# mlelarge/graph_neural_net

Measured on AMD Instinct MI355X. Metric: graph-pairs/sec FGNN fwd+bwd, N=50 regular pairs, higher is better.
Workload: dtype f32

## Files before the change

### graph_neural_net_amd/_lib.py

```python
import ctypes as C
import os

import torch

_HERE = os.path.dirname(os.path.abspath(__file__))
LIB_PATH = os.environ.get('FGNN_LIB') or os.path.join(_HERE, 'libfgnn_hip.so')

FGNN_H = 32
FGNN_TILE = 32
FGNN_MAX_DEPTH = 3
FGNN_RANGE_WG = 256
FGNN_LSAP_MAX_N = 2048
FGNN_QAP_MAX_N = 256
FGNN_SPECTRAL_MAX_N = 256
FGNN_SPECTRAL_MAX_POWERS = 8
FGNN_SCORE_SPLIT = 4

c_float_p = C.c_void_p


class Slab(C.Structure):
    _fields_ = [('ptr', C.c_void_p), ('gstride', C.c_longlong), ('ldp', C.c_longlong), ('C', C.c_int),
                ('nrm', C.c_void_p), ('beta', C.c_void_p)]


class MlpFwdArgs(C.Structure):
    _fields_ = [('G', C.c_int), ('N', C.c_int), ('depth', C.c_int), ('nmlp', C.c_int),
                ('nvalid', C.c_void_p),
                ('a', Slab), ('b', Slab),
                ('W', (C.c_void_p * FGNN_MAX_DEPTH) * 2),
                ('bias', (C.c_void_p * FGNN_MAX_DEPTH) * 2),
                ('z', C.c_void_p * 2),
                ('ldz', C.c_longlong),
                ('part', C.c_void_p * 2),
                ('cnt', C.c_void_p), ('packed', C.c_void_p), ('xbits', C.c_void_p), ('xdeg', C.c_void_p),
                ('ranges', C.c_void_p), ('cu_share', C.c_int)]


class DwJob(C.Structure):
    _fields_ = [('dy', C.c_void_p), ('d_gstride', C.c_longlong), ('d_ld', C.c_longlong), ('relu_mask', C.c_void_p),
                ('x', C.c_void_p), ('x_gstride', C.c_longlong), ('x_ld', C.c_longlong), ('M', C.c_int), ('K', C.c_int)]


class ChainLayer(C.Structure):
    _fields_ = [('W', C.c_void_p), ('w_ostride', C.c_longlong), ('w_kstride', C.c_longlong), ('bias', C.c_void_p),
                ('M', C.c_int), ('K', C.c_int), ('relu', C.c_int), ('mask', C.c_void_p), ('out', C.c_void_p),
                ('o_gstride', C.c_longlong)]


class ChainArgs(C.Structure):
    _fields_ = [('x', C.c_void_p), ('x_gstride', C.c_longlong), ('x_ld', C.c_longlong), ('depth', C.c_int),
                ('layer', ChainLayer * 3), ('o_ld', C.c_longlong), ('nvalid', C.c_void_p), ('G', C.c_int), ('N', C.c_int)]


class Mlp64Args(C.Structure):
    _fields_ = [('x', C.c_void_p), ('x_gstride', C.c_longlong), ('x_ld', C.c_longlong), ('cin', C.c_int),
                ('xb', C.c_void_p), ('xb_gstride', C.c_longlong), ('xb_ld', C.c_longlong), ('cb', C.c_int),
                ('packed', C.c_void_p), ('nvalid', C.c_void_p), ('G', C.c_int), ('N', C.c_int),
                ('out', C.c_void_p), ('o_gstride', C.c_longlong), ('o_ld', C.c_longlong),
                ('dz', C.c_void_p), ('dz_gstride', C.c_longlong), ('dz_ld', C.c_longlong),
                ('dx', C.c_void_p), ('dx_gstride', C.c_longlong), ('dx_ld', C.c_longlong),
                ('dxb', C.c_void_p), ('dxb_gstride', C.c_longlong), ('dxb_ld', C.c_longlong),
                ('accumulate_dx', C.c_int), ('accumulate_dxb', C.c_int),
                ('wpart', C.c_void_p)]


class Mlp64PackJob(C.Structure):
    _fields_ = [('W', C.c_void_p * 3), ('bias', C.c_void_p * 3), ('cin', C.c_int), ('packed', C.c_void_p)]


class MlpBwdArgs(C.Structure):
    _fields_ = [('G', C.c_int), ('N', C.c_int), ('depth', C.c_int),
                ('nvalid', C.c_void_p),
                ('a', Slab), ('b', Slab),
                ('W', C.c_void_p * FGNN_MAX_DEPTH),
                ('bias', C.c_void_p * FGNN_MAX_DEPTH),
                ('dy', C.c_void_p), ('dgstride', C.c_longlong), ('ldd', C.c_longlong),
                ('z', C.c_void_p), ('zgstride', C.c_longlong), ('ldz', C.c_longlong),
                ('coef', C.c_void_p), ('s12', C.c_void_p), ('znrm', C.c_void_p),
                ('dxa', C.c_void_p), ('dxa_gstride', C.c_longlong), ('dxa_ld', C.c_longlong),
                ('dxb', C.c_void_p), ('dxb_gstride', C.c_longlong), ('dxb_ld', C.c_longlong),
                ('accumulate_a', C.c_int), ('accumulate_b', C.c_int),
                ('wpart', C.c_void_p), ('s12part', C.c_void_p), ('packed', C.c_void_p),
                ('s12tiles', C.c_void_p), ('s12_out', C.c_void_p), ('xbits', C.c_void_p), ('xdeg', C.c_void_p),
                ('ranges', C.c_void_p), ('cu_share', C.c_int)]


class Slab16(C.Structure):
    _fields_ = [('ptr', C.c_void_p), ('gstride', C.c_longlong), ('ldp', C.c_longlong), ('C', C.c_int),
                ('nrm', C.c_void_p), ('beta', C.c_void_p)]


class MlpFwd16Args(C.Structure):
    _fields_ = [('G', C.c_int), ('N', C.c_int), ('ldr', C.c_int), ('depth', C.c_int), ('nmlp', C.c_int),
                ('nvalid', C.c_void_p),
                ('a', Slab16), ('b', Slab16),
                ('z', C.c_void_p * 2), ('ldz', C.c_longlong),
                ('part', C.c_void_p * 2), ('cnt', C.c_void_p), ('packed', C.c_void_p), ('ranges', C.c_void_p)]


class MlpBwd16Args(C.Structure):
    _fields_ = [('G', C.c_int), ('N', C.c_int), ('ldr', C.c_int), ('depth', C.c_int),
                ('nvalid', C.c_void_p),
                ('a', Slab16), ('b', Slab16),
                ('dy', C.c_void_p), ('dgstride', C.c_longlong), ('ldd', C.c_longlong),
                ('z', C.c_void_p), ('zgstride', C.c_longlong), ('ldz', C.c_longlong),
                ('coef', C.c_void_p),
                ('dxa', C.c_void_p), ('dxa_gstride', C.c_longlong), ('dxa_ld', C.c_longlong),
                ('dxb', C.c_void_p), ('dxb_gstride', C.c_longlong), ('dxb_ld', C.c_longlong),
                ('accumulate_a', C.c_int), ('accumulate_b', C.c_int),
                ('wpart', C.c_void_p), ('s12part', C.c_void_p), ('packed', C.c_void_p), ('ranges', C.c_void_p)]


class GradJob(C.Structure):
    _fields_ = [('wpart', C.c_void_p), ('count', C.c_int), ('out', C.c_void_p), ('s12', C.c_void_p),
                ('nrm', C.c_void_p), ('dgn_w', C.c_void_p), ('dgn_b', C.c_void_p), ('rows', C.c_int), ('scale', C.c_float), ('scale_dev', C.c_void_p)]


class PackJob(C.Structure):
    _fields_ = [('kind', C.c_int), ('ca', C.c_int), ('cb', C.c_int), ('depth', C.c_int), ('nmlp', C.c_int),
                ('W', (C.c_void_p * FGNN_MAX_DEPTH) * 2), ('bias', (C.c_void_p * FGNN_MAX_DEPTH) * 2),
                ('out', C.c_void_p)]


class PairgenArgs(C.Structure):
    _fields_ = [('seed', C.c_ulonglong), ('first', C.c_longlong), ('B', C.c_int), ('N', C.c_int),
                ('family', C.c_int), ('noise_model', C.c_int), ('edge_density', C.c_double),
                ('thr_edge', C.c_ulonglong), ('thr_noise1', C.c_ulonglong), ('thr_noise2', C.c_ulonglong),
                ('thr_vertex', C.c_ulonglong), ('swaps_per_edge', C.c_int),
                ('bits1', C.c_void_p), ('bits2', C.c_void_p), ('nvalid', C.c_void_p)]


MAX_GRAD_JOBS = 16
MAX_PACK_JOBS = 24
_VP, _LL, _I, _F = C.c_void_p, C.c_longlong, C.c_int, C.c_float

_SIGNATURES = {
    'fgnn_last_error': [],
    'fgnn_version': [],
    'fgnn_tiles_per_graph': [_I],
    'fgnn_mlp_bwd_num_workgroups': [],
    'fgnn_pack_floats': [_I, _I, _I, _I, _I],
    'fgnn_pack_operands': [_VP, _I, _VP],
    'fgnn_mlp_fwd': [C.POINTER(MlpFwdArgs), _VP],
    'fgnn_pack_x3_floats': [_I, _I, _I, _I, _I],
    'fgnn_pack_x3_operands': [_VP, _I, _VP],
    'fgnn_mlp_fwd_x3': [C.POINTER(MlpFwdArgs), _VP],
    'fgnn_debug_mlp_fwd_masks': [C.POINTER(MlpFwdArgs), _VP, _VP, _VP],
    'fgnn_debug_mlp_fwd_x3_masks': [C.POINTER(MlpFwdArgs), _VP, _VP, _VP],
    'fgnn_debug_matmul_variant': [_I],
    'fgnn_gn_finalize': [_VP, _VP, _VP, _VP, _I, _I, _I, _F, _VP, _VP],
    'fgnn_gn_finalize2': [_VP, _VP, _VP, _VP, _VP, _VP, _I, _I, _I, _F, _VP, _VP, _VP],
    'fgnn_gn_plane_supported': [_I],
    'fgnn_gn_plane_fwd': [_VP, _LL, _LL, _VP, _VP, _VP, _I, _I, _I, _F, _VP, _LL, _LL, _VP, _VP],
    'fgnn_gn_plane_bwd': [_VP, _LL, _LL, _VP, _LL, _LL, _VP, _VP, _I, _I, _I, _VP, _LL, _LL, _VP, _VP, _VP, _VP],
    'fgnn_gn_stats': [_VP, _LL, _LL, _VP, _VP, _I, _I, _I, _F, _VP, _VP],
    'fgnn_gn_apply': [_VP, _LL, _LL, _VP, _VP, _VP, _I, _I, _I, _VP, _LL, _LL, _VP],
    'fgnn_ragged_tile_ranges': [_VP, _I, _I, _VP, _VP],
    'fgnn_ragged_tile_ranges_order': [_VP, _I, _I, _VP, _VP, _VP],
    'fgnn_ragged_tile_ranges16': [_VP, _I, _I, _I, _VP, _VP],
    'fgnn_conv1x1_dw_multi': [C.POINTER(DwJob), _I, _VP, _I, _I, _VP, _VP],
    'fgnn_conv_chain_supported': [_I, _I, C.POINTER(C.c_int)],
    'fgnn_conv_chain': [C.POINTER(ChainArgs), _VP],
    'fgnn_mlp64_supported': [_I, _I, _I],
    'fgnn_mlp64_num_workgroups': [],
    'fgnn_mlp64_param_count': [_I],
    'fgnn_mlp64_packed_floats': [_I],
    'fgnn_mlp64_pack': [_VP, _VP, _VP, _VP, _VP, _VP, _I, _VP, _VP],
    'fgnn_mlp64_pack_multi': [C.POINTER(Mlp64PackJob), _I, _VP],
    'fgnn_mlp64_fwd': [C.POINTER(Mlp64Args), _VP],
    'fgnn_mlp64_bwd': [C.POINTER(Mlp64Args), _VP],
    'fgnn_conv1x1': [_VP, _LL, _LL, _VP, _VP, _LL, _LL, _VP, _I, _VP, _I, _I, _I, _I, _VP, _LL, _LL, _VP],
    'fgnn_conv1x1_dw_chunks': [_I, _I],
    'fgnn_conv1x1_dw': [_VP, _LL, _LL, _VP, _VP, _LL, _LL, _VP, _I, _I, _I, _I, _VP, _VP],
    'fgnn_chan_matmul_fwd': [C.POINTER(Slab), C.POINTER(Slab), _VP, _I, _I, _VP, _LL, _LL, _VP],
    'fgnn_chan_matmul_fwd_ord': [C.POINTER(Slab), C.POINTER(Slab), _VP, _I, _I, _VP, _LL, _LL, _VP, _I, _VP],
    'fgnn_chan_matmul_fwd_fin_supported': [_I],
    'fgnn_chan_matmul_fwd_fin': [C.POINTER(Slab), C.POINTER(Slab), _VP, _VP, _VP, _VP, _VP, _F, _VP, _I, _I, _VP, _LL, _LL, _VP],
    'fgnn_chan_matmul_fwd_fin_ord': [C.POINTER(Slab), C.POINTER(Slab), _VP, _VP, _VP, _VP, _VP, _F, _VP, _I, _I, _VP, _LL, _LL, _VP, _I, _VP],
    'fgnn_colmax_fwd': [C.POINTER(Slab), _VP, _I, _I, _VP, _VP, _VP],
    'fgnn_colmax_fwd_fin_supported': [_I],
    'fgnn_colmax_fwd_fin': [C.POINTER(Slab), _VP, _VP, _VP, _F, _VP, _I, _I, _VP, _VP, _VP],
    'fgnn_score_ce_fwd': [_VP, _VP, _VP, _I, _I, _I, _VP, _VP, _VP, _VP],
    'fgnn_score_row_blocks': [_I, _I],
    'fgnn_score_ce_fwd_blocks': [_VP, _VP, _VP, _I, _I, _I, _I, _VP, _VP, _VP, _VP],
    'fgnn_score_ce_bwd': [_VP, _VP, _VP, _VP, _VP, _VP, _I, _I, _I, _VP, _VP, _VP],
    'fgnn_inv_node_count': [_VP, _I, _VP, _VP],
    'fgnn_score_bwd': [_VP, _VP, _VP, _VP, _I, _I, _I, _VP, _VP, _VP],
    'fgnn_ce_fwd': [_VP, _VP, _I, _I, _VP, _VP, _VP],
    'fgnn_ce_bwd': [_VP, _VP, _VP, _VP, _I, _I, _VP, _VP],
    'fgnn_colmax_bwd': [_VP, _VP, _VP, _I, _I, _I, _VP, _LL, _LL, C.POINTER(Slab), _VP, _VP],
    'fgnn_gn_bwd_stats': [_VP, _LL, _LL, _VP, _LL, _LL, _VP, _VP, _I, _I, _I, _VP, _VP],
    'fgnn_gn_bwd_coef': [_VP, _VP, _VP, _I, _I, _I, _VP, _VP, _VP, _VP],
    'fgnn_gn_bwd_coef_tiles': [_VP, _VP, _VP, _I, _I, _I, _VP, _VP, _VP],
    'fgnn_grad_finalize': [_VP, _I, _I, _I, _I, _VP],
    'fgnn_gn_bwd_apply': [_VP, _LL, _LL, _VP, _LL, _LL, _VP, _VP, _I, _I, _I, _VP, _LL, _LL, _VP],
    'fgnn_mlp_bwd': [C.POINTER(MlpBwdArgs), _VP],
    'fgnn_mlp_bwd_x3': [C.POINTER(MlpBwdArgs), _VP],
    'fgnn_mlp_bwd_pair': [C.POINTER(MlpBwdArgs), C.POINTER(MlpBwdArgs), _VP],
    'fgnn_mlp_bwd_t16': [C.POINTER(MlpBwdArgs), _VP],
    'fgnn_mlp_bwd_t16_supported': [C.POINTER(MlpBwdArgs)],
    'fgnn_mlp_bwd_pair_t16': [C.POINTER(MlpBwdArgs), C.POINTER(MlpBwdArgs), _VP],
    'fgnn_mlp_bwd_pair_x3': [C.POINTER(MlpBwdArgs), C.POINTER(MlpBwdArgs), _VP],
    'fgnn_block1_struct_supported': [_I, _I, _I],
    'fgnn_block1_struct_table_floats': [_I],
    'fgnn_block1_struct_ws_floats': [_I, _I],
    'fgnn_block1_struct_rows': [_I, _I],
    'fgnn_block1_struct_fwd': [_VP, _VP, _I, _I, _VP, _VP, _VP, _VP, _VP, C.c_float, _VP, _VP, _VP, _LL, _LL, _VP, _VP, _VP, _VP, _VP, _VP, _VP],
    'fgnn_block1_struct_bwd': [_VP, _VP, _I, _I, _VP, _VP, _VP, _VP, _VP, _VP, _VP, _VP, _LL, _LL, _VP, _VP, _VP, _VP, _VP, _VP],
    'fgnn_block1_struct_fwd_pack': [_VP, _VP, _I, _I, _VP, _VP, _VP, _VP, _VP, C.c_float, _VP, _VP, _VP, _LL, _LL, _VP, _VP, _VP, _VP, _VP, _VP, _VP, _I, _VP],
    'fgnn_block1_struct_fwd16_pack': [_VP, _VP, _I, _I, _I, _VP, _VP, _VP, _VP, _VP, C.c_float, _VP, _VP, _VP, _LL, _LL, _VP, _VP, _VP, _VP, _VP, _VP, _VP, _I, _VP],
    'fgnn_block1_struct_fwd16': [_VP, _VP, _I, _I, _I, _VP, _VP, _VP, _VP, _VP, C.c_float, _VP, _VP, _VP, _LL, _LL, _VP, _VP, _VP, _VP, _VP, _VP, _VP],
    'fgnn_block1_struct_bwd16': [_VP, _VP, _I, _I, _I, _VP, _VP, _VP, _VP, _VP, _VP, _VP, _VP, _LL, _LL, _VP, _VP, _VP, _VP, _VP, _VP],
    'fgnn_mlp_bwd_coef_tiles_supported': [_I, _I],
    'fgnn_mlp_param_count': [_I, _I],
    'fgnn_reduce_partials': [_VP, _I, _I, _VP, _VP],
    'fgnn_chan_matmul_bwd': [C.POINTER(Slab), C.POINTER(Slab), _VP, _LL, _LL, _VP, _I, _I, _VP, _VP, _LL, _LL, _VP, _VP, _VP],
    'fgnn_chan_matmul_bwd_ord': [C.POINTER(Slab), C.POINTER(Slab), _VP, _LL, _LL, _VP, _I, _I, _VP, _VP, _LL, _LL, _VP, _VP, _VP, _I, _VP],
    'fgnn_sum_scale': [_VP, _I, _I, _F, _VP, _VP],
    'fgnn_adam_step': [_VP, _VP, _VP, _VP, _I, C.c_double, C.c_double, C.c_double, C.c_double, _I, C.c_double, _VP],
    'fgnn_adam_step_dev': [_VP, _VP, _VP, _VP, _I, _VP, _VP, _VP],
    'fgnn_expand_adjacency': [_VP, _VP, _I, _I, _VP, _VP],
    'fgnn_pack_adjacency': [_VP, _VP, _I, _I, _VP, _VP, _VP],
    'fgnn_pack_adjacency_ld': [_VP, _VP, _I, _I, _I, _VP, _VP, _VP],
    'fgnn_pack_adjacency_pair': [_VP, _VP, _VP, _VP, _I, _I, _I, _VP, _VP, _VP, _VP, _VP],
    'fgnn_adjacency_degree': [_VP, _VP, _I, _I, _VP, _VP],
    'fgnn_accuracy_max': [_VP, _VP, _I, _I, _VP, _VP],
    'fgnn_lsap_accuracy': [_VP, _LL, _I, _VP, _I, _I, _VP, _VP, _VP],
    'fgnn_pairgen_supported': [_I, _I, _I],
    'fgnn_pairgen': [C.POINTER(PairgenArgs), _VP],
    'fgnn_qap_objective': [_VP, _VP, _VP, _VP, _I, _I, _VP, _VP, _VP, _VP, _VP],
    'fgnn_qap_improve_cost': [_VP, _VP, _VP, _VP, _I, _I, _VP, _LL, _I, _VP],
    'fgnn_greedy_qap_ws_bytes': [_I, _I],
    'fgnn_greedy_qap': [_VP, _VP, _VP, _VP, _I, _I, _I, _VP, _LL, _VP, _VP, _VP, _VP, _VP],
    'fgnn_spectral_features': [_VP, _VP, _I, _I, _I, _VP, _I, _VP],
    'fgnn_tiles_per_graph16': [_I, _I],
    'fgnn_to_bf16': [_VP, _VP, _I, _I, _I, _I, _VP, _LL, _LL, _VP],
    'fgnn_from_bf16': [_VP, _LL, _LL, _I, _I, _I, _I, _VP, _VP],
    'fgnn_pack16_floats': [_I, _I, _I, _I, _I],
    'fgnn_pack16_operands': [_VP, _I, _VP],
    'fgnn_mlp_fwd16': [C.POINTER(MlpFwd16Args), _VP],
    'fgnn_debug_mlp_fwd16_masks': [C.POINTER(MlpFwd16Args), _VP, _VP, _VP],
    'fgnn_gn_finalize_tpg': [_VP, _VP, _VP, _VP, _I, _I, _I, _I, _F, _VP, _VP],
    'fgnn_gn_finalize2_tpg': [_VP, _VP, _VP, _VP, _VP, _VP, _I, _I, _I, _I, _F, _VP, _VP, _VP],
    'fgnn_gn_bwd_coef_tiles_tpg': [_VP, _VP, _VP, _I, _I, _I, _I, _VP, _VP, _VP],
    'fgnn_chan_matmul_fwd16': [C.POINTER(Slab16), C.POINTER(Slab16), _VP, _I, _I, _I, _VP, _LL, _LL, _VP],
    'fgnn_chan_matmul_fwd16_fin': [C.POINTER(Slab16), C.POINTER(Slab16), _VP, _VP, _VP, _VP, _VP, _F, _I, _VP, _I, _I, _I, _VP, _LL,
                                   _LL, _VP],
    'fgnn_chan_matmul_bwd16': [C.POINTER(Slab16), C.POINTER(Slab16), _VP, _LL, _LL, _VP, _I, _I, _I, _VP, _VP, _LL, _LL, _VP, _VP, _VP],
    'fgnn_chan_matmul_bwd16_t': [C.POINTER(Slab16), C.POINTER(Slab16), _VP, _LL, _LL, _VP, _I, _VP, _I, _I, _I, _VP, _VP, _LL, _LL,
                                 _VP, _VP, _VP],
    'fgnn_chan_matmul_bwd16_tc': [C.POINTER(Slab16), C.POINTER(Slab16), _VP, _LL, _LL, _VP, _I, _VP, _I, _I, _I, _VP, _VP, _LL, _LL,
                                  _VP, _VP, _VP, _VP, _VP],
    'fgnn_colmax_bwd16_coef': [_VP, _VP, _VP, _I, _I, _I, _I, _VP, _LL, _LL, C.POINTER(Slab16), _VP, _VP, _VP],
    'fgnn_colmax_fwd16': [C.POINTER(Slab16), _VP, _I, _I, _I, _VP, _VP, _VP],
    'fgnn_colmax_bwd16': [_VP, _VP, _VP, _I, _I, _I, _I, _VP, _LL, _LL, C.POINTER(Slab16), _VP, _VP],
    'fgnn_mlp_bwd16': [C.POINTER(MlpBwd16Args), _VP],
    'fgnn_mlp_bwd16_pair': [C.POINTER(MlpBwd16Args), C.POINTER(MlpBwd16Args), _VP],
}
_RESTYPES = {'fgnn_last_error': C.c_char_p, 'fgnn_block1_struct_ws_floats': C.c_longlong, 'fgnn_greedy_qap_ws_bytes': C.c_longlong}
EXPORTS = tuple(_SIGNATURES)

_lib = None


def load():
    global _lib
    if _lib is not None:
        return _lib
    if not os.path.exists(LIB_PATH):
        raise RuntimeError(
            'graph_neural_net_amd: %s is missing. Build it with '
            '`python -c "import __graft_entry__ as g; g.build()"` or `make -C graph_neural_net_amd/csrc`. '
            'There is no CPU fallback.' % LIB_PATH)
    lib = C.CDLL(LIB_PATH)
    for name, argtypes in _SIGNATURES.items():
        fn = getattr(lib, name)
        fn.argtypes = argtypes
        fn.restype = _RESTYPES.get(name, C.c_int)
    _lib = lib
    return lib


def last_error():
    return load().fgnn_last_error().decode('utf-8', 'replace')


PROFILE = None


def call(name, *args, tag=None):
    if PROFILE is not None:
        e0 = torch.cuda.Event(enable_timing=True)
        e1 = torch.cuda.Event(enable_timing=True)
        e0.record()
        rc = getattr(load(), name)(*args)
        e1.record()
        PROFILE.append((tag or name, e0, e1, name, args))
    else:
        rc = getattr(load(), name)(*args)
    if rc != 0:
        raise RuntimeError('%s failed (rc=%d): %s' % (name, rc, last_error()))


def relaunch(name, args):
    rc = getattr(load(), name)(*args[:-1], stream_ptr())
    if rc != 0:
        raise RuntimeError('%s failed (rc=%d): %s' % (name, rc, last_error()))


def stream_ptr():
    return C.c_void_p(torch.cuda.current_stream().cuda_stream)


def ptr(t):
    if t is None:
        return None
    if not t.is_cuda:
        raise RuntimeError('graph_neural_net_amd: expected a CUDA/HIP tensor, got device %s '
                           '(there is no CPU path)' % (t.device,))
    return C.c_void_p(t.data_ptr())


def make_slab(t, gstride, ldp, channels, nrm=None, beta=None):
    s = Slab()
    s.ptr = t.data_ptr() if t is not None else None
    s.gstride = gstride
    s.ldp = ldp
    s.C = channels
    s.nrm = nrm.data_ptr() if nrm is not None else None
    s.beta = beta.data_ptr() if beta is not None else None
    return s


def make_slab16(t, gstride, ldp, channels, nrm=None, beta=None):
    s = Slab16()
    s.ptr = t.data_ptr() if t is not None else None
    s.gstride = gstride
    s.ldp = ldp
    s.C = channels
    s.nrm = nrm.data_ptr() if nrm is not None else None
    s.beta = beta if isinstance(beta, int) else (beta.data_ptr() if beta is not None else None)
    return s


def tiles_per_graph(n):
    return (n * n + FGNN_TILE - 1) // FGNN_TILE


def mlp_param_count(cin, depth):
    return 32 * cin + 32 + (depth - 1) * (32 * 32 + 32)
```

### graph_neural_net_amd/csrc/mlp_bwd_t16.hip

```cpp
#include "fgnn_t16.h"
#include "fgnn_pack.h"

namespace {

using namespace t16;

constexpr int BWD_WG = 256;
constexpr int NW = 8;

DEVI float4 coef_from_sums(const float4 n, const float2 sv, float nv) {
    const float m = nv * nv;
    float4 k;
    k.x = n.x;
    k.y = n.y;
    k.z = m > 0.f ? -n.y * sv.y * n.w / m : 0.f;
    k.w = m > 0.f ? -n.y * sv.x / m : 0.f;
    return k;
}
DEVI int graph_nv(const rsrc_t &rnv, bool ragged, int g, int N) {
    const int v = __builtin_amdgcn_raw_buffer_load_b32(rnv, g * 4, 0, 0);
    return __builtin_amdgcn_readfirstlane(ragged ? v : N);
}

template <int CB>
struct Layout16 {
    static constexpr int DEPTH = 3;
    static constexpr PkBwd PK = pk_bwd(32, CB, DEPTH);
    static constexpr int OFF_W0A = PK.off_w1a, OFF_W0B = PK.off_w1b, OFF_W1 = PK.off_wh, OFF_WT1 = PK.off_wt, OFF_WT2 = PK.off_wt + 16;
    static constexpr int OFF_WT0A = PK.off_wt0a, OFF_WT0B = PK.off_wt0b;
    static constexpr int BIAS_F = PK.bias_f;
    static constexpr int WEIGHT_F = pk_pad_floats(PK.floats);
    static constexpr int NSLOT = 5;
    static constexpr int CIN = 32 + CB;
    static constexpr int PCOUNT = 32 * CIN + 32 + (DEPTH - 1) * (32 * 32 + 32);
    static constexpr int TILE_OFF = WEIGHT_F;
    static constexpr int REC_OFF = TILE_OFF + NW * NSLOT * TILE_F;
    static constexpr int WGK_OFF = REC_OFF + NW * 256;
    static constexpr int LIVE_OFF = WGK_OFF + FGNN_BWD_COEF_GRAPHS * 128;
    static constexpr int MAIN_F = LIVE_OFF + LIVE_LIST_CAP + NW;
    static constexpr int RED_F = NW * PCOUNT;
    static constexpr int LDS_F = MAIN_F > RED_F ? MAIN_F : RED_F;
};

template <int CB, bool PKD, bool SKIP, bool DXB>
__global__ __launch_bounds__(64 * NW, 2) void mlp_bwd_t16_kernel(const fgnn_mlp_bwd_args A, const int tpg, const int total_tiles) {
    extern __shared__ __attribute__((aligned(16))) float smem[];
    using L = Layout16<CB>;
    constexpr bool NB = CB == 32;
    const int lane = threadIdx.x & 63, wv = __builtin_amdgcn_readfirstlane(threadIdx.x >> 6);
    const int px = lane & 15, q = lane >> 4;
    const int P2 = A.N * A.N, hpg = 2 * tpg;
    const View va = make_view(A.a.ptr, A.a.gstride, A.a.ldp, A.G);
    const View vb = make_view(A.b.ptr, A.b.gstride, A.b.ldp, A.G);
    PackedSrc ps = {};
    if constexpr (PKD) ps = make_packed_src(A.xbits, A.xdeg, A.G, A.N);
    const View vdy = make_view(A.dy, A.dgstride, A.ldd, A.G);
    const View vz = make_view(A.z, A.zgstride, A.ldz, A.G);
    const View vdxa = make_view(A.dxa, A.dxa_gstride, A.dxa_ld, A.G);
    const View vdxb = make_view(A.dxb, A.dxb_gstride, A.dxb_ld, A.G);

    float *wl = smem;
    float *my = smem + L::TILE_OFF + wv * (L::NSLOT * TILE_F);
    float *XA = my, *XB = my + TILE_F, *S0 = my + 2 * TILE_F, *S1 = my + 3 * TILE_F, *S2 = my + 4 * TILE_F;
    const int lane_base = tile_lane_base(px, q);

    f32x4 dW0a[4], dW0b[4], dW1[4], dW2[4];
    float db0[2] = {0.f, 0.f}, db1[2] = {0.f, 0.f}, db2[2] = {0.f, 0.f}, dbx[2] = {0.f, 0.f};
#pragma unroll
    for (int k = 0; k < 4; ++k) dW0a[k] = dW0b[k] = dW1[k] = dW2[k] = zero4();

    const int nwg = gridDim.x;
    const int qq = total_tiles / nwg, rem = total_tiles % nwg;
    int T0 = blockIdx.x * qq + ((int)blockIdx.x < rem ? (int)blockIdx.x : rem);
    int T1 = T0 + qq + ((int)blockIdx.x < rem ? 1 : 0);
    if constexpr (SKIP) {
        T0 = A.ranges[blockIdx.x];
        T1 = A.ranges[blockIdx.x + 1];
    }
    const int H0 = 2 * T0, H1 = 2 * T1;
    const bool ragged = A.nvalid != nullptr;
    const rsrc_t rnv = __builtin_amdgcn_make_buffer_rsrc(const_cast<int *>(A.nvalid), 0, ragged ? A.G * 4 : 0, 0x00020000);
    const float rcpN = 1.f / (float)A.N;
    const bool from_tiles = A.s12tiles != nullptr;
    const int g0 = T0 / tpg;
    float4 *wgK = reinterpret_cast<float4 *>(smem + L::WGK_OFF);

    int live_cnt = 0;
    int *live_list = reinterpret_cast<int *>(smem + L::LIVE_OFF);
    int nlive = 0, lk = wv - NW;
    bool use_list = false;
    if constexpr (SKIP) {
        nlive = build_live_list(live_list, live_list + LIVE_LIST_CAP, T0, T1, tpg, FGNN_TILE, A.N, A.nvalid, threadIdx.x, 64 * NW);
        use_list = nlive <= LIVE_LIST_CAP;
    }
    auto next_half = [&](int h) {
        if constexpr (SKIP) {
            if (use_list) {
                int r = H1;
                while (true) {
                    lk += NW;
                    if ((lk >> 1) >= nlive) break;
                    const int t = live_list[lk >> 1], g = t / tpg, hh = 2 * (t - g * tpg) + (lk & 1);
                    if (hh * 16 < P2) {
                        r = 2 * t + (lk & 1);
                        break;
                    }
                }
                return __builtin_amdgcn_readfirstlane(r);
            }
            while (h < H1) {
                const int g = h / hpg, hh = h - g * hpg;
                const int nv = A.nvalid[g];
                if (hh * 16 < P2 && tile_live(hh >> 1, A.N, nv)) {
                    const bool mine = live_cnt % NW == wv;
                    ++live_cnt;
                    if (mine) break;
                    ++h;
                } else if ((hh >> 1) * FGNN_TILE / A.N >= nv) {
                    h = (g + 1) * hpg;
                } else {
                    ++h;
                }
            }
            return __builtin_amdgcn_readfirstlane(h < H1 ? h : H1);
        } else {
            while (h < H1) {
                const int g = h / hpg, hh = h - g * hpg;
                if (hh * 16 < P2) break;
                h += NW;
            }
            return __builtin_amdgcn_readfirstlane(h);
        }
    };

    pk_glds<NW>(smem, A.packed, L::WEIGHT_F, wv, lane);

    float mean[8], av[8], beta[8], kx[8], ky[8], kz[8], kw[8];
#pragma unroll
    for (int s = 0; s < 8; ++s) {
        mean[s] = 0.f;
        av[s] = 1.f;
        beta[s] = (NB && A.b.nrm && A.b.beta) ? A.b.beta[chan_s(s) + chan_q(q)] : 0.f;
        kx[s] = ky[s] = kz[s] = kw[s] = 0.f;
    }
    float4 *rec = reinterpret_cast<float4 *>(smem + L::REC_OFF) + wv * 64;
    auto fetch_records = [&](int g, int nv) {
        if (lane < 32) {
            float4 k4;
            if (from_tiles) k4 = wgK[(g - g0) * 32 + lane];
            else if (A.coef) k4 = reinterpret_cast<const float4 *>(A.coef)[(long long)g * FGNN_H + lane];
            else {
                const float4 n = reinterpret_cast<const float4 *>(A.znrm)[(long long)g * FGNN_H + lane];
                const float2 sv = reinterpret_cast<const float2 *>(A.s12)[(long long)g * FGNN_H + lane];
                k4 = coef_from_sums(n, sv, (float)nv);
            }
            rec[lane] = k4;
            if (NB && A.b.nrm) rec[32 + lane] = reinterpret_cast<const float4 *>(A.b.nrm)[(long long)g * A.b.C + lane];
        }
    };
    auto read_records = [&]() {
#pragma unroll
        for (int s = 0; s < 8; ++s) {
            const float4 k4 = rec[chan_s(s) + chan_q(q)];
            kx[s] = k4.x;
            ky[s] = k4.y;
            kz[s] = k4.z;
            kw[s] = k4.w;
            if (NB && A.b.nrm) {
                const float4 n = rec[32 + chan_s(s) + chan_q(q)];
                mean[s] = n.x;
                av[s] = n.y;
            }
        }
    };

    constexpr int NXB = CB == 32 ? 8 : 1;
    float xa[8], xb[NXB], dyr[8], zr[8];
    auto load_x = [&](int h) {
        const bool act = h < H1;
        const int g = __builtin_amdgcn_readfirstlane(act ? h / hpg : 0);
        const int p = (act ? h - g * hpg : 0) * 16 + px;
        const bool inb = act && p < P2;
        load8(xa, va, lane_voff(va, q, p, inb), g * va.gs4);
        if constexpr (CB == 32) {
            load8(xb, vb, lane_voff(vb, q, p, inb), g * vb.gs4);
        } else if constexpr (PKD) {
            int i, jj;
            row_col(p, A.N, rcpN, i, jj);
            const int ob = (inb && q == 0) ? (i * ps.words + (jj >> 5)) * 4 : OOB_OFF;
            const int od = (inb && q == 1 && i == jj) ? i * 4 : OOB_OFF;
            const unsigned w = (unsigned)__builtin_amdgcn_raw_buffer_load_b32(ps.bits, ob, g * ps.N * ps.words * 4, 0);
            const float d = __builtin_bit_cast(float, __builtin_amdgcn_raw_buffer_load_b32(ps.deg, od, g * ps.N * 4, 0));
            xb[0] = q == 0 ? (((w >> (jj & 31)) & 1u) ? 1.f : 0.f) : d;
        } else {
            xb[0] = buf_load(vb, (inb && q < 2) ? q * vb.ld4 + 4 * p : OOB_OFF, g * vb.gs4);
        }
    };
    auto load_dyz = [&](int h) {
        const bool act = h < H1;
        const int g = __builtin_amdgcn_readfirstlane(act ? h / hpg : 0);
        const int p = (act ? h - g * hpg : 0) * 16 + px;
        const bool inb = act && p < P2;
        load8(dyr, vdy, lane_voff(vdy, q, p, inb), g * vdy.gs4);
        load8(zr, vz, lane_voff(vz, q, p, inb), g * vz.gs4);
    };

    int h = next_half(SKIP ? H0 : H0 + wv);
    load_x(h);
    int cached_g = -1, cur_nv = A.N;

    if (from_tiles) {
        const int g1 = T1 > T0 ? (T1 - 1) / tpg : g0 - 1;
        float2 *scr = reinterpret_cast<float2 *>(smem + L::TILE_OFF);
        const int cc = threadIdx.x & 31, sl = threadIdx.x >> 5;
        for (int g = g0; g <= g1; ++g) {
            float p1 = 0.f, p2 = 0.f;
            constexpr int TS = (64 * NW) / 32, U = 8;
            for (int t0 = sl; t0 < tpg; t0 += TS * U) {
                float2 v[U];
#pragma unroll
                for (int k = 0; k < U; ++k) {
                    const int t = t0 + TS * k;
                    v[k] = reinterpret_cast<const float2 *>(A.s12tiles)[((long long)g * tpg + (t < tpg ? t : 0)) * FGNN_H + cc];
                }
#pragma unroll
                for (int k = 0; k < U; ++k) {
                    if (t0 + TS * k < tpg) {
                        p1 += v[k].x;
                        p2 += v[k].y;
                    }
                }
            }
            scr[sl * 32 + cc] = make_float2(p1, p2);
            __syncthreads();
            if (threadIdx.x < 32) {
                float s1 = 0.f, s2 = 0.f;
#pragma unroll
                for (int k = 0; k < (64 * NW) / 32; ++k) {
                    s1 += scr[k * 32 + cc].x;
                    s2 += scr[k * 32 + cc].y;
                }
                const float2 sv = make_float2(s1, s2);
                if (A.s12_out) reinterpret_cast<float2 *>(A.s12_out)[(long long)g * FGNN_H + cc] = sv;
                const float4 n = reinterpret_cast<const float4 *>(A.znrm)[(long long)g * FGNN_H + cc];
                wgK[(g - g0) * 32 + cc] = coef_from_sums(n, sv, (float)graph_nv(rnv, ragged, g, A.N));
            }
            __syncthreads();
        }
    }
    if (h < H1) {
        const int g = h / hpg;
        cur_nv = graph_nv(rnv, ragged, g, A.N);
        fetch_records(g, cur_nv);
        cached_g = g;
    }
    if constexpr (CB == 2) {
        for (int e = lane; e < 16 * TLD; e += 64) XB[e] = 0.f;
    }
    __syncthreads();
    load_dyz(h);
    if (cached_g >= 0) read_records();

    while (h < H1) {
        const int hn = next_half(SKIP ? h + 1 : h + NW);
        const int g = __builtin_amdgcn_readfirstlane(h / hpg), hh = h - g * hpg;
        const int p = hh * 16 + px;
        const bool inb = p < P2;
        if (g != cached_g) {
            cur_nv = graph_nv(rnv, ragged, g, A.N);
            fetch_records(g, cur_nv);
            read_records();
            cached_g = g;
        }
        bool valid = inb;
        if (ragged) {
            int i, jj;
            row_col(p, A.N, rcpN, i, jj);
            valid = inb && i < cur_nv && jj < cur_nv;
        }
        const bool full = __ballot(valid) == ~0ull;

        float h1[8], h2[8];
        {
            float yb[NXB];
            if constexpr (NB) {
#pragma unroll
                for (int s = 0; s < 8; ++s) yb[s] = (xb[s] - mean[s]) * av[s] + beta[s];
            } else {
                yb[0] = xb[0];
            }
            stage8(XA, lane_base, xa);
            if constexpr (CB == 32) {
                stage8(XB, lane_base, yb);
            } else {
                if (q < 2) XB[8 * q * TLD + px] = yb[0];
            }
            f32x4 acc[2];
            load_bias(acc, wl + L::BIAS_F, 0, q);
            gemm32<L::OFF_W0A>(acc, wl, xa, lane);
            if constexpr (CB == 32) gemm32<L::OFF_W0B>(acc, wl, yb, lane);
            else gemm2<L::OFF_W0B>(acc, wl, q < 2 ? yb[0] : 0.f, lane);
            load_x(hn);
#pragma unroll
            for (int s = 0; s < 8; ++s) h1[s] = relu1(acc[s >> 2][s & 3]);
            stage8(S0, lane_base, h1);
            load_bias(acc, wl + L::BIAS_F, 1, q);
            gemm32<L::OFF_W1>(acc, wl, h1, lane);
#pragma unroll
            for (int s = 0; s < 8; ++s) h2[s] = relu1(acc[s >> 2][s & 3]);
            stage8(S1, lane_base, h2);
        }
        float dpre[8];
#pragma unroll
        for (int s = 0; s < 8; ++s) dpre[s] = fmaf(kz[s], zr[s] - kx[s], fmaf(ky[s], dyr[s], kw[s]));
        if (!full) {
#pragma unroll
            for (int s = 0; s < 8; ++s) dpre[s] = valid ? dpre[s] : 0.f;
        }
        stage8(S2, lane_base, dpre);
        load_dyz(hn);
        __builtin_amdgcn_sched_barrier(0);
        {
            f32x4 a2[2];
            a2[0] = a2[1] = zero4();
            gemm32<L::OFF_WT2>(a2, wl, dpre, lane);
            wgrad16(dW2, db2, S2, S1, lane);
#pragma unroll
            for (int s = 0; s < 8; ++s) dpre[s] = h2[s] > 0.f ? a2[s >> 2][s & 3] : 0.f;
        }
        __builtin_amdgcn_sched_barrier(0);
        stage8(S1, lane_base, dpre);
        {
            f32x4 a2[2];
            a2[0] = a2[1] = zero4();
            gemm32<L::OFF_WT1>(a2, wl, dpre, lane);
            wgrad16(dW1, db1, S1, S0, lane);
#pragma unroll
            for (int s = 0; s < 8; ++s) dpre[s] = h1[s] > 0.f ? a2[s >> 2][s & 3] : 0.f;
        }
        __builtin_amdgcn_sched_barrier(0);
        stage8(S2, lane_base, dpre);
        __builtin_amdgcn_sched_barrier(0);
        {
            f32x4 dx[2];
            float v[8];
            dx[0] = dx[1] = zero4();
            gemm32<L::OFF_WT0A>(dx, wl, dpre, lane);
            wgrad16(dW0a, db0, S2, XA, lane);
#pragma unroll
            for (int s = 0; s < 8; ++s) v[s] = dx[s >> 2][s & 3];
            store8(v, vdxa, lane_voff(vdxa, q, p, inb), g * vdxa.gs4);
            if constexpr (DXB) {
                dx[0] = dx[1] = zero4();
                gemm32<L::OFF_WT0B>(dx, wl, dpre, lane);
            }
            if constexpr (CB == 32) {
                wgrad16(dW0b, dbx, S2, XB, lane);
            } else {
                const int i = lane & 15;
                const float4 a0 = *reinterpret_cast<const float4 *>(S2 + i * TLD + 4 * q);
                const float4 a1 = *reinterpret_cast<const float4 *>(S2 + (16 + i) * TLD + 4 * q);
                const float4 b0 = *reinterpret_cast<const float4 *>(XB + i * TLD + 4 * q);
                dW0b[0] = mfma16(a0.x, b0.x, dW0b[0]);
                dW0b[2] = mfma16(a1.x, b0.x, dW0b[2]);
                dW0b[0] = mfma16(a0.y, b0.y, dW0b[0]);
                dW0b[2] = mfma16(a1.y, b0.y, dW0b[2]);
                dW0b[0] = mfma16(a0.z, b0.z, dW0b[0]);
                dW0b[2] = mfma16(a1.z, b0.z, dW0b[2]);
                dW0b[0] = mfma16(a0.w, b0.w, dW0b[0]);
                dW0b[2] = mfma16(a1.w, b0.w, dW0b[2]);
            }
            if constexpr (DXB) {
#pragma unroll
                for (int s = 0; s < 8; ++s) v[s] = dx[s >> 2][s & 3];
                store8(v, vdxb, lane_voff(vdxb, q, p, inb), g * vdxb.gs4);
            }
        }
        h = hn;
    }

    constexpr int PCOUNT = L::PCOUNT, CIN = L::CIN;
#pragma unroll
    for (int b = 0; b < 2; ++b) {
        db0[b] += __shfl_xor(db0[b], 16);
        db0[b] += __shfl_xor(db0[b], 32);
        db1[b] += __shfl_xor(db1[b], 16);
        db1[b] += __shfl_xor(db1[b], 32);
        db2[b] += __shfl_xor(db2[b], 16);
        db2[b] += __shfl_xor(db2[b], 32);
    }
    (void)dbx;
    __syncthreads();
    {
        float *red = smem + wv * PCOUNT;
#pragma unroll
        for (int mb = 0; mb < 2; ++mb)
#pragma unroll
            for (int nb = 0; nb < 2; ++nb)
#pragma unroll
                for (int r = 0; r < 4; ++r) {
                    const int o = row_chan(16 * mb + 4 * q + r), c = row_chan(16 * nb + px);
                    red[o * CIN + c] = dW0a[2 * mb + nb][r];
                    if (c < CB) red[o * CIN + 32 + c] = dW0b[2 * mb + nb][r];
                    red[32 * CIN + 32 + o * 32 + c] = dW1[2 * mb + nb][r];
                    red[32 * CIN + 32 + 1056 + o * 32 + c] = dW2[2 * mb + nb][r];
                }
        if (q == 0) {
            const int c0 = row_chan(px), c1 = row_chan(16 + px);
            red[32 * CIN + c0] = db0[0];
            red[32 * CIN + c1] = db0[1];
            red[32 * CIN + 32 + 1024 + c0] = db1[0];
            red[32 * CIN + 32 + 1024 + c1] = db1[1];
            red[32 * CIN + 32 + 1056 + 1024 + c0] = db2[0];
            red[32 * CIN + 32 + 1056 + 1024 + c1] = db2[1];
        }
    }
    __syncthreads();
    static_assert(PCOUNT % 4 == 0, "partials are summed four at a time");
    float4 *out = reinterpret_cast<float4 *>(A.wpart + (long long)blockIdx.x * PCOUNT);
    const float4 *part4 = reinterpret_cast<const float4 *>(smem);
    for (int e = threadIdx.x; e < PCOUNT / 4; e += 64 * NW) {
        float4 a = part4[e];
#pragma unroll
        for (int w = 1; w < NW; ++w) {
            const float4 b = part4[w * (PCOUNT / 4) + e];
            a.x += b.x;
            a.y += b.y;
            a.z += b.z;
            a.w += b.w;
        }
        out[e] = a;
    }
}

template <int CB, bool PKD, bool SKIP, bool DXB>
int launch16(const fgnn_mlp_bwd_args *a, int tpg, int total, hipStream_t st) {
    constexpr int LDS = Layout16<CB>::LDS_F * 4;
    static_assert(LDS <= 160 * 1024, "LDS budget");
    static LdsAttrCache attr_cache;
    (void)fgnn_raise_lds(attr_cache, (const void *)mlp_bwd_t16_kernel<CB, PKD, SKIP, DXB>, LDS);
    hipLaunchKernelGGL((mlp_bwd_t16_kernel<CB, PKD, SKIP, DXB>), dim3(a->cu_share == 2 && !SKIP ? BWD_WG / 2 : BWD_WG), dim3(64 * NW), LDS, st, *a,
                       tpg, total);
    FGNN_LAUNCH_CHECK();
    return 0;
}
template <int CB, bool PKD, bool DXB>
int launch16s(const fgnn_mlp_bwd_args *a, int tpg, int total, hipStream_t st) {
    return a->ranges ? launch16<CB, PKD, true, DXB>(a, tpg, total, st) : launch16<CB, PKD, false, DXB>(a, tpg, total, st);
}

}

extern "C" int fgnn_mlp_bwd_t16_supported(const fgnn_mlp_bwd_args *a) {
    if (!a || a->depth != 3 || a->a.C != 32 || a->a.nrm || !a->dxa || a->accumulate_a || a->accumulate_b || !a->packed || a->N > 256) return 0;
    if (a->b.C == 32) return (a->b.nrm && a->dxb && !a->xbits) ? 1 : 0;
    if (a->b.C == 2) return (!a->b.nrm && !a->dxb) ? 1 : 0;
    return 0;
}

extern "C" int fgnn_mlp_bwd_t16(const fgnn_mlp_bwd_args *a, void *stream) {
    FGNN_CHECK(a != nullptr, "fgnn_mlp_bwd_t16: null args");
    FGNN_CHECK(fgnn_mlp_bwd_t16_supported(a), "fgnn_mlp_bwd_t16: built for depth 3, slab a = 32 raw channels with dx stored, slab b = 32 normalised "
               "channels with dx stored or 2 raw channels without dx, an operand image of kind 5, N <= 256; use fgnn_mlp_bwd");
    FGNN_CHECK(a->G > 0 && a->N > 0 && a->a.ptr && (a->b.ptr || (a->xbits && a->b.C == 2)), "fgnn_mlp_bwd_t16: bad G / N / slabs");
    FGNN_CHECK(!a->xbits || a->xdeg, "fgnn_mlp_bwd_t16: xbits without xdeg (fgnn_adjacency_degree)");
    FGNN_CHECK(a->dy && a->z && a->wpart, "fgnn_mlp_bwd_t16: missing dy/z/wpart");
    FGNN_CHECK(a->coef || (a->s12 && a->znrm) || (a->s12tiles && a->znrm), "fgnn_mlp_bwd_t16: need coef, or s12 + znrm, or s12tiles + znrm");
    FGNN_CHECK(BWD_WG == fgnn_mlp_bwd_num_workgroups() && BWD_WG == FGNN_RANGE_WG, "fgnn_mlp_bwd_t16: workgroup count differs from fgnn_mlp_bwd");
    {
        const long long lim = 0x7fffffffll / 4, G = a->G;
        FGNN_CHECK(G * a->a.gstride < lim && G * a->b.gstride < lim && G * a->dgstride < lim && G * a->zgstride < lim &&
                   G * a->dxa_gstride < lim && G * a->dxb_gstride < lim,
                   "fgnn_mlp_bwd_t16: a tensor exceeds 2 GiB (32-bit buffer addressing); split the batch");
    }
    for (int l = 0; l < a->depth; ++l) FGNN_CHECK(a->W[l] && a->bias[l], "fgnn_mlp_bwd_t16: missing weights layer %d", l);
    const int tpg = fgnn_tiles_per_graph(a->N);
    const long long total = (long long)a->G * tpg;
    FGNN_CHECK(total < (1ll << 29), "fgnn_mlp_bwd_t16: too many tiles");
    FGNN_CHECK(!a->ranges || (a->nvalid && !a->s12tiles), "fgnn_mlp_bwd_t16: ranges need nvalid and exclude s12tiles");
    FGNN_CHECK(!a->s12tiles || fgnn_mlp_bwd_coef_tiles_supported(a->G, a->N), "fgnn_mlp_bwd_t16: s12tiles needs a workgroup's tile range to span <= %d graphs",
               FGNN_BWD_COEF_GRAPHS);
    hipStream_t st = (hipStream_t)stream;
    if (a->b.C == 32) return launch16s<32, false, true>(a, tpg, (int)total, st);
    if (a->xbits) return launch16s<2, true, false>(a, tpg, (int)total, st);
    return launch16s<2, false, false>(a, tpg, (int)total, st);
}
```

### graph_neural_net_amd/csrc/pool_score.hip

```cpp
#include <float.h>
#include "fgnn_common.h"
#include "fgnn_norm.h"

namespace {

__global__ __launch_bounds__(256) void colmax_fwd_kernel(const fgnn_slab y, const int *nvalid, int G, int N, float *e,
                                                         int *idx) {
    const long long t = (long long)blockIdx.x * (blockDim.x / WAVE) + (threadIdx.x / WAVE);
    const int C = y.C;
    if (t >= (long long)G * C * N) return;
    const int lane = threadIdx.x & 63;
    const int i = (int)(t % N);
    const int gc = (int)(t / N);
    const int g = gc / C, c = gc - g * C;
    const int nv = nvalid_of(nvalid, g, N);
    float best = 0.f;
    int bi = 0;
    if (i < nv) {
        const float *row = y.ptr + (long long)g * y.gstride + (long long)c * y.ldp + (long long)i * N;
        float mean = 0.f, a = 1.f, be = 0.f;
        if (y.nrm) {
            const float4 n = reinterpret_cast<const float4 *>(y.nrm)[gc];
            mean = n.x;
            a = n.y;
            be = y.beta ? y.beta[c] : 0.f;
        }
        best = -FLT_MAX;
        bi = 0x7fffffff;
        for (int j = lane; j < nv; j += WAVE) {
            float v = row[j];
            if (y.nrm) v = (v - mean) * a + be;
            if (v > best) {
                best = v;
                bi = j;
            }
        }
        for (int o = 32; o > 0; o >>= 1) {
            const float ov = __shfl_xor(best, o);
            const int oi = __shfl_xor(bi, o);
            if (ov > best || (ov == best && oi < bi)) {
                best = ov;
                bi = oi;
            }
        }
    }
    if (lane == 0) {
        e[t] = best;
        idx[t] = bi;
    }
}

template <int KC>
struct __attribute__((packed, aligned(4))) ColFloats {
    float v[KC];
};
template <int KC>
__global__ __launch_bounds__(256) void colmax_fwd_rows16_kernel(const fgnn_slab y, const int *nvalid, int G, int N, float *e, int *idx) {
    const int lane = threadIdx.x & 63, sub = lane & 15;
    const long long t = ((long long)blockIdx.x * 4 + (threadIdx.x >> 6)) * 4 + (lane >> 4);
    const int C = y.C;
    const bool live = t < (long long)G * C * N;
    const long long tc = live ? t : 0;
    const int i = (int)(tc % N);
    const int gc = (int)(tc / N);
    const int g = gc / C, c = gc - g * C;
    const int nv = nvalid_of(nvalid, g, N);
    float best = 0.f;
    int bi = 0;
    if (live && i < nv) {
        const float *row = y.ptr + (long long)g * y.gstride + (long long)c * y.ldp + (long long)i * N;
        float mean = 0.f, a = 1.f, be = 0.f;
        if (y.nrm) {
            const float4 n = reinterpret_cast<const float4 *>(y.nrm)[gc];
            mean = n.x;
            a = n.y;
            be = y.beta ? y.beta[c] : 0.f;
        }
        const int j0 = KC * sub;
        float v[KC];
        if (j0 + KC <= N) {
            const ColFloats<KC> f = *reinterpret_cast<const ColFloats<KC> *>(row + j0);
#pragma unroll
            for (int k = 0; k < KC; ++k) v[k] = f.v[k];
        } else {
#pragma unroll
            for (int k = 0; k < KC; ++k) v[k] = j0 + k < N ? row[j0 + k] : 0.f;
        }
        best = -FLT_MAX;
        bi = 0x7fffffff;
#pragma unroll
        for (int k = 0; k < KC; ++k) {
            const float x = y.nrm ? (v[k] - mean) * a + be : v[k];
            if (j0 + k < nv && x > best) {
                best = x;
                bi = j0 + k;
            }
        }
    }
#define FGNN_COLMAX_STEP(CTRL)                                                                                         \
    {                                                                                                                  \
        const float ov = dpp_mov<CTRL>(best);                                                                          \
        const int oi = __builtin_amdgcn_update_dpp(0, bi, CTRL, 0xf, 0xf, true);                                       \
        if (ov > best || (ov == best && oi < bi)) {                                                                    \
            best = ov;                                                                                                 \
            bi = oi;                                                                                                   \
        }                                                                                                              \
    }
    FGNN_COLMAX_STEP(0xB1)
    FGNN_COLMAX_STEP(0x4E)
    FGNN_COLMAX_STEP(0x141)
    FGNN_COLMAX_STEP(0x140)
#undef FGNN_COLMAX_STEP
    if (live && sub == 0) {
        e[t] = i < nv ? best : 0.f;
        idx[t] = i < nv ? bi : 0;
    }
}

struct ColmaxFin {
    const float *part, *cnt, *gw;
    float eps;
    int tpg;
};
template <bool FIN>
__global__ __launch_bounds__(256) void colmax_fwd_lds_kernel(const fgnn_slab y, const int *nvalid, int G, int N,
                                                             float *e, int *idx, const ColmaxFin F) {
    __shared__ float sm[4][64 * 65];
    const int wave = threadIdx.x >> 6, lane = threadIdx.x & 63;
    const int gc = xcd_swizzle(blockIdx.x, gridDim.x) * 4 + wave;
    const int C = y.C;
    if (gc >= G * C) return;
    const int g = gc / C, c = gc - g * C;
    const int nv = nvalid_of(nvalid, g, N);
    const float *mat = y.ptr + (long long)g * y.gstride + (long long)c * y.ldp;
    float mean = 0.f, a = 1.f, be = 0.f;
    TilePartials tp;
    if (FIN) tp = finalize_load(F.part, F.cnt, g, c, C, F.tpg, lane);
    float x[64];
    const int col = lane < N ? lane : 0;
#pragma unroll
    for (int q = 0; q < 8; ++q) {
        if (8 * q < N) {
#pragma unroll
            for (int r = 0; r < 8; ++r) {
                const int i = 8 * q + r;
                x[i] = mat[(i < N ? i : 0) * N + col];
            }
        }
    }
    if (FIN) {
        const float4 n = finalize_reduce(tp, (float)nv, F.gw ? F.gw[c] : 1.f, F.eps);
        if (lane == 0) reinterpret_cast<float4 *>(const_cast<float *>(y.nrm))[gc] = n;
        mean = n.x;
        a = n.y;
        be = y.beta ? y.beta[c] : 0.f;
    } else if (y.nrm) {
        const float4 n = reinterpret_cast<const float4 *>(y.nrm)[gc];
        mean = n.x;
        a = n.y;
        be = y.beta ? y.beta[c] : 0.f;
    }
    float *t = sm[wave];
    const int ld = N + 1;
    const bool norm = FIN || y.nrm;
    if (lane < N) {
#pragma unroll
        for (int q = 0; q < 8; ++q) {
            if (8 * q < N) {
#pragma unroll
                for (int r = 0; r < 8; ++r) {
                    const int i = 8 * q + r;
                    if (i < N) t[i * ld + lane] = norm ? (x[i] - mean) * a + be : x[i];
                }
            }
        }
    }
    float best = 0.f;
    int bi = 0;
    if (lane < nv) {
        best = -FLT_MAX;
        const float *row = t + lane * ld;
        for (int jj = 0; jj < nv; ++jj) {
            const float v = row[jj];
            if (v > best) {
                best = v;
                bi = jj;
            }
        }
    }
    if (lane < N) {
        e[(long long)gc * N + lane] = best;
        idx[(long long)gc * N + lane] = bi;
    }
}

constexpr int CMB_MAXN = 1024;
__global__ __launch_bounds__(256) void colmax_bwd_kernel(const float *de, const int *idx, const int *nvalid, int G, int C,
                                                         int N, float *dy, long long gstride, long long ldp,
                                                         const fgnn_slab y, float *s12) {
    __shared__ int sidx[CMB_MAXN];
    __shared__ float sde[CMB_MAXN];
    __shared__ float red[4][2];
    const int gc = blockIdx.x, tid = threadIdx.x, lane = tid & 63, wave = tid >> 6;
    const int g = gc / C, c = gc - g * C;
    const int nv = nvalid_of(nvalid, g, N);
    float *mat = dy + (long long)g * gstride + (long long)c * ldp;
    const float *zm = s12 ? y.ptr + (long long)g * y.gstride + (long long)c * y.ldp : nullptr;
    const float mean = s12 ? y.nrm[(long long)gc * 4] : 0.f;
    const bool staged = N <= CMB_MAXN;
    float s1 = 0.f, s2 = 0.f;
    const bool late = N <= 256;
    float zlate = 0.f, dlate = 0.f;
    for (int i = tid; i < N; i += 256) {
        const long long t = (long long)gc * N + i;
        const int bi = idx[t];
        const float d = i < nv ? de[t] : 0.f;
        if (staged) {
            sidx[i] = bi;
            sde[i] = d;
        }
        if (s12 && i < nv) {
            if (late) {
                zlate = zm[(long long)i * N + bi];
                dlate = d;
            } else {
                s1 += d;
                s2 += d * (zm[(long long)i * N + bi] - mean);
            }
        }
    }
    __syncthreads();
    const float invN = 1.f / (float)N;
    if (staged && (ldp & 3) == 0 && (gstride & 3) == 0 && (reinterpret_cast<unsigned long long>(dy) & 15ull) == 0) {
        const int P = N * N;
        float4 *mat4 = reinterpret_cast<float4 *>(mat);
        for (int q = tid; 4 * q < P; q += 256) {
            const int p0 = 4 * q;
            int i = (int)(((float)p0 + 0.5f) * invN);
            int j = p0 - i * N;
            float v[4];
#pragma unroll
            for (int k = 0; k < 4; ++k) {
                const int ic = i < N ? i : 0;
                v[k] = (i < N && j == sidx[ic]) ? sde[ic] : 0.f;
                if (++j == N) {
                    j = 0;
                    ++i;
                }
            }
            if (p0 + 3 < P) {
                mat4[q] = make_float4(v[0], v[1], v[2], v[3]);
            } else {
#pragma unroll
                for (int k = 0; k < 4; ++k)
                    if (p0 + k < P) mat[p0 + k] = v[k];
            }
        }
    } else {
        for (int p = tid; p < N * N; p += 256) {
            const int i = (int)(((float)p + 0.5f) * invN);
            const int j = p - i * N;
            const int bi = staged ? sidx[i] : idx[(long long)gc * N + i];
            const float d = staged ? sde[i] : (i < nv ? de[(long long)gc * N + i] : 0.f);
            mat[p] = (j == bi) ? d : 0.f;
        }
    }
    if (s12) {
        if (late && tid < nv) {
            s1 += dlate;
            s2 += dlate * (zlate - mean);
        }
        s1 = wave_sum(s1);
        s2 = wave_sum(s2);
        if (lane == 0) {
            red[wave][0] = s1;
            red[wave][1] = s2;
        }
        __syncthreads();
        if (tid < 2) s12[(long long)gc * 2 + tid] = (red[0][tid] + red[1][tid]) + (red[2][tid] + red[3][tid]);
    }
}

DEVI void copy_to_lds256(float *dst, const float *src, int n, int tid) {
    constexpr int U = 8;
    int done = 0;
    if (((reinterpret_cast<unsigned long long>(src) | reinterpret_cast<unsigned long long>(dst)) & 15ull) == 0) {
        const int n4 = n >> 2;
        const float4 *s4 = reinterpret_cast<const float4 *>(src);
        float4 *d4 = reinterpret_cast<float4 *>(dst);
        for (int e0 = tid; e0 < n4; e0 += 256 * U) {
            float4 v[U];
#pragma unroll
            for (int k = 0; k < U; ++k) {
                const int e = e0 + 256 * k;
                v[k] = s4[e < n4 ? e : 0];
            }
#pragma unroll
            for (int k = 0; k < U; ++k) {
                const int e = e0 + 256 * k;
                if (e < n4) d4[e] = v[k];
            }
        }
        done = n4 << 2;
    }
    for (int e0 = done + tid; e0 < n; e0 += 256 * U) {
        float v[U];
#pragma unroll
        for (int k = 0; k < U; ++k) {
            const int e = e0 + 256 * k;
            v[k] = src[e < n ? e : 0];
        }
#pragma unroll
        for (int k = 0; k < U; ++k) {
            const int e = e0 + 256 * k;
            if (e < n) dst[e] = v[k];
        }
    }
}

__global__ __launch_bounds__(256) void score_ce_fwd_kernel(const float *e1, const float *e2, const int *nvalid,
                                                           int C, int N, int rows, float *scores, float *lse,
                                                           float *pair_loss) {
    extern __shared__ __attribute__((aligned(16))) float sm[];
    float *s2 = sm, *s1 = sm + (size_t)C * N;
    float *sS = s1 + (size_t)C * rows;
    float *red = sS + (size_t)rows * N;
    const int b = blockIdx.x, tid = threadIdx.x, lane = tid & 63, wave = tid >> 6;
    const int nv = nvalid_of(nvalid, b, N);
    const int i0 = blockIdx.y * rows;
    const int i1 = (i0 + rows < N) ? i0 + rows : N;
    const int w = i1 > i0 ? i1 - i0 : 0;
    const float *p1 = e1 + (long long)b * C * N, *p2 = e2 + (long long)b * C * N;
    copy_to_lds256(s2, p2, C * N, tid);
    for (int e = tid; e < C * w; e += 256) {
        const int c = e / w, r = e - c * w;
        s1[c * rows + r] = p1[c * N + i0 + r];
    }
    __syncthreads();
    float *S = scores + (long long)b * N * N;
    const float invN = 1.f / (float)N;
    for (int e = tid; e < w * N; e += 256) {
        const int r = (int)(((float)e + 0.5f) * invN), j = e - r * N;
        float acc = 0.f;
        if (i0 + r < nv && j < nv)
            for (int c = 0; c < C; ++c) acc = fmaf(s1[c * rows + r], s2[c * N + j], acc);
        S[(long long)i0 * N + e] = acc;
        sS[e] = acc;
    }
    __syncthreads();
    float wl = 0.f;
    for (int i = i0 + wave; i < i1; i += 4) {
        float l = 0.f;
        const float *Sr = sS + (size_t)(i - i0) * N;
        if (i < nv) {
            float mx = -FLT_MAX;
            for (int j = lane; j < nv; j += WAVE) mx = fmaxf(mx, Sr[j]);
            mx = wave_max(mx);
            float se = 0.f;
            for (int j = lane; j < nv; j += WAVE) se += expf(Sr[j] - mx);
            se = wave_sum(se);
            l = mx + logf(se);
            wl += l - Sr[i];
        }
        if (lane == 0 && lse) lse[(long long)b * N + i] = l;
    }
    if (lane == 0) red[wave] = wl;
    __syncthreads();
    if (tid == 0 && pair_loss) pair_loss[b * gridDim.y + blockIdx.y] = (red[0] + red[1]) + (red[2] + red[3]);
}

constexpr int CSPLIT = 4;
constexpr int CSPLIT_SMALL = 8;
template <bool CE, bool STAGE>
__global__ __launch_bounds__(256) void score_bwd_kernel(const float *e1, const float *e2, const float *scores,
                                                        const float *lse, const float *dscores, const int *nvalid,
                                                        const float *gscale, int C, int N, float *de1, float *de2) {
    extern __shared__ __attribute__((aligned(16))) float sm[];
    const int cper = (C + (int)gridDim.y - 1) / (int)gridDim.y;
    const int c0 = blockIdx.y * cper;
    const int cn = (c0 + cper <= C ? cper : (C > c0 ? C - c0 : 0));
    float *s1 = sm, *s2 = sm + (size_t)cper * N;
    float *dS = s2 + (size_t)cper * N;
    const int ld = N + 1;
    const int b = blockIdx.x, tid = threadIdx.x;
    const int nv = nvalid_of(nvalid, b, N);
    const float *p1 = e1 + ((long long)b * C + c0) * N, *p2 = e2 + ((long long)b * C + c0) * N;
    for (int e = tid; e < cn * N; e += 256) {
        s1[e] = p1[e];
        s2[e] = p2[e];
    }
    const float gs = CE ? *gscale : 1.f;
    const float *S = (CE ? scores : dscores) + (long long)b * N * N;
    const float *Lr = CE ? lse + (long long)b * N : nullptr;
    const float invN = 1.f / (float)N;
    auto ds_at = [&](int i, int jj) -> float {
        float d = S[(long long)i * N + jj];
        if (CE) d = (expf(d - Lr[i]) - (i == jj ? 1.f : 0.f)) * gs;
        return d;
    };
    if (STAGE) {
        constexpr int U = 8;
        for (int e0 = tid; e0 < N * N; e0 += 256 * U) {
            float v[U];
#pragma unroll
            for (int k = 0; k < U; ++k) {
                const int e = e0 + 256 * k;
                v[k] = S[e < N * N ? e : 0];
            }
#pragma unroll
            for (int k = 0; k < U; ++k) {
                const int e = e0 + 256 * k;
                if (e < N * N) {
                    const int i = (int)(((float)e + 0.5f) * invN);
                    const int jj = e - i * N;
                    float d = 0.f;
                    if (i < nv && jj < nv) {
                        d = v[k];
                        if (CE) d = (expf(d - Lr[i]) - (i == jj ? 1.f : 0.f)) * gs;
                    }
                    dS[i * ld + jj] = d;
                }
            }
        }
    }
    __syncthreads();
    for (int e = tid; e < cn * N; e += 256) {
        const int c = e / N, i = e - c * N;
        float a1 = 0.f, a2 = 0.f;
        if (i < nv) {
            const float *r2 = s2 + c * N, *r1 = s1 + c * N;
            for (int jj = 0; jj < nv; ++jj) {
                a1 = fmaf(r2[jj], STAGE ? dS[i * ld + jj] : ds_at(i, jj), a1);
                a2 = fmaf(r1[jj], STAGE ? dS[jj * ld + i] : ds_at(jj, i), a2);
            }
        }
        de1[((long long)b * C + c0) * N + e] = a1;
        de2[((long long)b * C + c0) * N + e] = a2;
    }
}

template <bool CE>
__global__ __launch_bounds__(256) void score_bwd_blocked_kernel(const float *e1, const float *e2, const float *scores,
                                                                const float *lse, const float *dscores,
                                                                const int *nvalid, const float *gscale, int C, int N,
                                                                int SB_BLK, float *de1, float *de2) {
    extern __shared__ __attribute__((aligned(16))) float sm[];
    const int cper = (C + CSPLIT - 1) / CSPLIT;
    const int c0 = blockIdx.y * cper;
    const int cn = (c0 + cper <= C ? cper : (C > c0 ? C - c0 : 0));
    float *s1 = sm, *s2 = sm + (size_t)cper * N;
    float *dS = s2 + (size_t)cper * N;
    const int b = blockIdx.x, tid = threadIdx.x;
    const int nv = nvalid_of(nvalid, b, N);
    const int x0 = blockIdx.z * SB_BLK, x1 = (x0 + SB_BLK < N) ? x0 + SB_BLK : N, w = x1 - x0;
    const float *p1 = e1 + ((long long)b * C + c0) * N, *p2 = e2 + ((long long)b * C + c0) * N;
    constexpr int U = 8;
    copy_to_lds256(s1, p1, cn * N, tid);
    copy_to_lds256(s2, p2, cn * N, tid);
    const float gs = CE ? *gscale : 1.f;
    const float *S = (CE ? scores : dscores) + (long long)b * N * N;
    const float *Lr = CE ? lse + (long long)b * N : nullptr;
    auto ds_of = [&](float sv, float lv, int i, int jj) -> float {
        if (i >= nv || jj >= nv) return 0.f;
        return CE ? (expf(sv - lv) - (i == jj ? 1.f : 0.f)) * gs : sv;
    };
    {
        const int ld = N + 1;
        for (int e0 = tid; e0 < w * N; e0 += 256 * U) {
            float sv[U], lv[U];
#pragma unroll
            for (int k = 0; k < U; ++k) {
                const int e = e0 + 256 * k, ec = e < w * N ? e : 0;
                const int r = ec / N;
                sv[k] = S[(long long)x0 * N + ec];
                lv[k] = CE ? Lr[x0 + r] : 0.f;
            }
#pragma unroll
            for (int k = 0; k < U; ++k) {
                const int e = e0 + 256 * k;
                if (e < w * N) {
                    const int r = e / N, jj = e - r * N;
                    dS[r * ld + jj] = ds_of(sv[k], lv[k], x0 + r, jj);
                }
            }
        }
        __syncthreads();
        for (int e = tid; e < cn * w; e += 256) {
            const int c = e / w, r = e - c * w;
            float a1 = 0.f;
            const float *r2 = s2 + c * N, *drow = dS + r * ld;
            for (int jj = 0; jj < nv; ++jj) a1 = fmaf(r2[jj], drow[jj], a1);
            de1[((long long)b * C + c0 + c) * N + x0 + r] = (x0 + r) < nv ? a1 : 0.f;
        }
        __syncthreads();
    }
    {
        const int ld = SB_BLK + 1;
        for (int e0 = tid; e0 < N * w; e0 += 256 * U) {
            float sv[U], lv[U];
#pragma unroll
            for (int k = 0; k < U; ++k) {
                const int e = e0 + 256 * k, ec = e < N * w ? e : 0;
                const int i = ec / w, r = ec - i * w;
                sv[k] = S[(long long)i * N + x0 + r];
                lv[k] = CE ? Lr[i] : 0.f;
            }
#pragma unroll
            for (int k = 0; k < U; ++k) {
                const int e = e0 + 256 * k;
                if (e < N * w) {
                    const int i = e / w, r = e - i * w;
                    dS[i * ld + r] = ds_of(sv[k], lv[k], i, x0 + r);
                }
            }
        }
        __syncthreads();
        for (int e = tid; e < cn * w; e += 256) {
            const int c = e / w, r = e - c * w;
            float a2 = 0.f;
            const float *r1 = s1 + c * N;
            for (int i = 0; i < nv; ++i) a2 = fmaf(r1[i], dS[i * ld + r], a2);
            de2[((long long)b * C + c0 + c) * N + x0 + r] = (x0 + r) < nv ? a2 : 0.f;
        }
    }
}

__global__ __launch_bounds__(256) void ce_fwd_kernel(const float *scores, const int *nvalid, int N, float *lse,
                                                     float *pair_loss) {
    __shared__ float red[4];
    const int b = blockIdx.x, tid = threadIdx.x, lane = tid & 63, wave = tid >> 6;
    const int nv = nvalid_of(nvalid, b, N);
    const float *S = scores + (long long)b * N * N;
    float wl = 0.f;
    for (int i = wave; i < N; i += 4) {
        float l = 0.f;
        if (i < nv) {
            float mx = -FLT_MAX;
            for (int j = lane; j < nv; j += WAVE) mx = fmaxf(mx, S[(long long)i * N + j]);
            mx = wave_max(mx);
            float se = 0.f;
            for (int j = lane; j < nv; j += WAVE) se += expf(S[(long long)i * N + j] - mx);
            se = wave_sum(se);
            l = mx + logf(se);
            wl += l - S[(long long)i * N + i];
        }
        if (lane == 0 && lse) lse[(long long)b * N + i] = l;
    }
    if (lane == 0) red[wave] = wl;
    __syncthreads();
    if (tid == 0 && pair_loss) pair_loss[b] = (red[0] + red[1]) + (red[2] + red[3]);
}

__global__ void ce_bwd_kernel(const float *scores, const float *lse, const int *nvalid, const float *gscale, int N,
                              float *dscores) {
    const int b = blockIdx.y;
    const int e = blockIdx.x * blockDim.x + threadIdx.x;
    if (e >= N * N) return;
    const int nv = nvalid_of(nvalid, b, N);
    const int i = e / N, j = e - i * N;
    float d = 0.f;
    if (i < nv && j < nv)
        d = (expf(scores[(long long)b * N * N + e] - lse[(long long)b * N + i]) - (i == j ? 1.f : 0.f)) * (*gscale);
    dscores[(long long)b * N * N + e] = d;
}

}

extern "C" int fgnn_colmax_fwd(const fgnn_slab *y, const int *nvalid, int G, int N, float *e, int *idx, void *stream) {
    FGNN_CHECK(y && y->ptr && e && idx && G > 0 && N > 0 && y->C > 0, "fgnn_colmax_fwd: bad arguments");
    const long long tot = (long long)G * y->C * N;
    if (N <= 64) {
        hipLaunchKernelGGL(colmax_fwd_lds_kernel<false>, dim3((unsigned)((G * y->C + 3) / 4)), dim3(256), 0,
                           (hipStream_t)stream, *y, nvalid, G, N, e, idx, ColmaxFin{});
        FGNN_LAUNCH_CHECK();
        return 0;
    }
    if (N <= 128) {
        hipLaunchKernelGGL(colmax_fwd_rows16_kernel<8>, dim3((unsigned)((tot + 15) / 16)), dim3(256), 0, (hipStream_t)stream, *y, nvalid, G, N, e, idx);
        FGNN_LAUNCH_CHECK();
        return 0;
    }
    if (N <= 256) {
        hipLaunchKernelGGL(colmax_fwd_rows16_kernel<16>, dim3((unsigned)((tot + 15) / 16)), dim3(256), 0, (hipStream_t)stream, *y, nvalid, G, N, e, idx);
        FGNN_LAUNCH_CHECK();
        return 0;
    }
    hipLaunchKernelGGL(colmax_fwd_kernel, dim3((unsigned)((tot + 3) / 4)), dim3(256), 0, (hipStream_t)stream, *y,
                       nvalid, G, N, e, idx);
    FGNN_LAUNCH_CHECK();
    return 0;
}

extern "C" int fgnn_colmax_fwd_fin_supported(int N) { return N <= 64 ? 1 : 0; }

extern "C" int fgnn_colmax_fwd_fin(const fgnn_slab *y, const float *part, const float *cnt, const float *gn_weight, float eps,
                                   const int *nvalid, int G, int N, float *e, int *idx, void *stream) {
    FGNN_CHECK(y && y->ptr && y->nrm && part && cnt && e && idx && G > 0 && N > 0 && y->C > 0, "fgnn_colmax_fwd_fin: bad arguments");
    FGNN_CHECK(N <= 64, "fgnn_colmax_fwd_fin: N=%d > 64 (use fgnn_gn_finalize + fgnn_colmax_fwd)", N);
    const ColmaxFin F = {part, cnt, gn_weight, eps, fgnn_tiles_per_graph(N)};
    hipLaunchKernelGGL(colmax_fwd_lds_kernel<true>, dim3((unsigned)((G * y->C + 3) / 4)), dim3(256), 0, (hipStream_t)stream, *y,
                       nvalid, G, N, e, idx, F);
    FGNN_LAUNCH_CHECK();
    return 0;
}

extern "C" int fgnn_colmax_bwd(const float *de, const int *idx, const int *nvalid, int G, int C, int N, float *dy,
                               long long gstride, long long ldp, const fgnn_slab *y, float *s12, void *stream) {
    FGNN_CHECK(de && idx && dy && G > 0 && C > 0 && N > 0, "fgnn_colmax_bwd: bad arguments");
    FGNN_CHECK(!s12 || (y && y->ptr && y->nrm && y->C == C), "fgnn_colmax_bwd: s12 needs the normalised input slab");
    fgnn_slab ys = {};
    if (s12) ys = *y;
    const int tot = G * C;
    hipLaunchKernelGGL(colmax_bwd_kernel, dim3((unsigned)tot), dim3(256), 0, (hipStream_t)stream, de,
                       idx, nvalid, G, C, N, dy, gstride, ldp, ys, s12);
    FGNN_LAUNCH_CHECK();
    return 0;
}

static int score_lds_bytes(int C, int N) { return (2 * C * N + 4) * (int)sizeof(float); }
static int score_bwd_lds_bytes(int C, int N, bool stage, int csplit = CSPLIT) {
    const int cper = (C + csplit - 1) / csplit;
    return (2 * cper * N + (stage ? N * (N + 1) : 0)) * (int)sizeof(float);
}
template <bool CE>
static int launch_score_bwd(const float *e1, const float *e2, const float *scores, const float *lse,
                            const float *dscores, const int *nvalid, const float *gscale, int B, int C, int N,
                            float *de1, float *de2, hipStream_t st) {
    const bool stage = score_bwd_lds_bytes(C, N, true) <= 160 * 1024 && (N <= 64 || (long long)B * CSPLIT >= 256);
    const int csplit = (long long)B * CSPLIT < 256 ? CSPLIT_SMALL : CSPLIT;
    const int lds = score_bwd_lds_bytes(C, N, stage, stage ? csplit : CSPLIT);
    FGNN_CHECK(lds <= 160 * 1024, "score backward: C*N=%d too large for LDS staging", C * N);
    if (stage) {
        if (lds > 64 * 1024)
            (void)hipFuncSetAttribute((const void *)score_bwd_kernel<CE, true>, hipFuncAttributeMaxDynamicSharedMemorySize, lds);
        hipLaunchKernelGGL((score_bwd_kernel<CE, true>), dim3(B, csplit), dim3(256), lds, st, e1, e2, scores, lse, dscores,
                           nvalid, gscale, C, N, de1, de2);
    } else {
        const int cper = (C + CSPLIT - 1) / CSPLIT;
        const int SB_BLK = (long long)B * CSPLIT * ((N + 63) / 64) >= 512 ? 64 : 16;
        const int big = (N + 1) * SB_BLK > N * (SB_BLK + 1) ? (N + 1) * SB_BLK : N * (SB_BLK + 1);
        const int lds2 = (2 * cper * N + big) * (int)sizeof(float);
        FGNN_CHECK(lds2 <= 160 * 1024, "score backward: N=%d too large for the blocked LDS staging", N);
        if (lds2 > 64 * 1024)
            (void)hipFuncSetAttribute((const void *)score_bwd_blocked_kernel<CE>, hipFuncAttributeMaxDynamicSharedMemorySize, lds2);
        hipLaunchKernelGGL((score_bwd_blocked_kernel<CE>), dim3(B, CSPLIT, (N + SB_BLK - 1) / SB_BLK), dim3(256), lds2, st, e1, e2,
                           scores, lse, dscores, nvalid, gscale, C, N, SB_BLK, de1, de2);
    }
    FGNN_LAUNCH_CHECK();
    return 0;
}

extern "C" int fgnn_score_row_blocks(int B, int N) {
    if (B * FGNN_SCORE_SPLIT >= 512) return FGNN_SCORE_SPLIT;
    return (N + 3) / 4;
}

extern "C" int fgnn_score_ce_fwd_blocks(const float *e1, const float *e2, const int *nvalid, int B, int C, int N,
                                        int row_blocks, float *scores, float *lse, float *pair_loss, void *stream) {
    FGNN_CHECK(e1 && e2 && scores && B > 0 && C > 0 && N > 0 && row_blocks > 0, "fgnn_score_ce_fwd: bad arguments");
    const int rows = (N + row_blocks - 1) / row_blocks;
    const int lds = (C * N + C * rows + rows * N + 4) * (int)sizeof(float);
    FGNN_CHECK(lds <= 160 * 1024, "fgnn_score_ce_fwd: C*N=%d too large for LDS staging", C * N);
    if (lds > 64 * 1024)
        (void)hipFuncSetAttribute((const void *)score_ce_fwd_kernel, hipFuncAttributeMaxDynamicSharedMemorySize, lds);
    hipLaunchKernelGGL(score_ce_fwd_kernel, dim3(B, row_blocks), dim3(256), lds, (hipStream_t)stream, e1, e2, nvalid, C, N, rows,
                       scores, lse, pair_loss);
    FGNN_LAUNCH_CHECK();
    return 0;
}

extern "C" int fgnn_score_ce_fwd(const float *e1, const float *e2, const int *nvalid, int B, int C, int N,
                                 float *scores, float *lse, float *pair_loss, void *stream) {
    return fgnn_score_ce_fwd_blocks(e1, e2, nvalid, B, C, N, FGNN_SCORE_SPLIT, scores, lse, pair_loss, stream);
}

extern "C" int fgnn_score_ce_bwd(const float *e1, const float *e2, const float *scores, const float *lse,
                                 const int *nvalid, const float *gscale, int B, int C, int N, float *de1, float *de2,
                                 void *stream) {
    FGNN_CHECK(e1 && e2 && scores && lse && gscale && de1 && de2 && B > 0, "fgnn_score_ce_bwd: bad arguments");
    return launch_score_bwd<true>(e1, e2, scores, lse, nullptr, nvalid, gscale, B, C, N, de1, de2, (hipStream_t)stream);
}

extern "C" int fgnn_score_bwd(const float *e1, const float *e2, const float *dscores, const int *nvalid, int B, int C,
                              int N, float *de1, float *de2, void *stream) {
    FGNN_CHECK(e1 && e2 && dscores && de1 && de2 && B > 0, "fgnn_score_bwd: bad arguments");
    return launch_score_bwd<false>(e1, e2, nullptr, nullptr, dscores, nvalid, nullptr, B, C, N, de1, de2, (hipStream_t)stream);
}

extern "C" int fgnn_ce_fwd(const float *scores, const int *nvalid, int B, int N, float *lse, float *pair_loss,
                           void *stream) {
    FGNN_CHECK(scores && lse && pair_loss && B > 0 && N > 0, "fgnn_ce_fwd: bad arguments");
    hipLaunchKernelGGL(ce_fwd_kernel, dim3(B), dim3(256), 0, (hipStream_t)stream, scores, nvalid, N, lse, pair_loss);
    FGNN_LAUNCH_CHECK();
    return 0;
}

extern "C" int fgnn_ce_bwd(const float *scores, const float *lse, const int *nvalid, const float *gscale, int B, int N,
                           float *dscores, void *stream) {
    FGNN_CHECK(scores && lse && gscale && dscores && B > 0 && N > 0, "fgnn_ce_bwd: bad arguments");
    hipLaunchKernelGGL(ce_bwd_kernel, dim3((N * N + 255) / 256, B), dim3(256), 0, (hipStream_t)stream, scores, lse,
                       nvalid, gscale, N, dscores);
    FGNN_LAUNCH_CHECK();
    return 0;
}
```

### graph_neural_net_amd/engine.py

```python
import ctypes as C
import os

import torch

from . import _lib
from .engine_base import EngineBase

EPS = 1e-05


class ParamLayout:

    def __init__(self, original_features_num=2, num_blocks=4, in_features=32, out_features=32, depth_of_mlp=3):
        if in_features != _lib.FGNN_H or out_features != _lib.FGNN_H:
            raise RuntimeError('the fused engine is built for in_features = out_features = 32 (got %d, %d); other widths '
                               'run through the per-layer modules (layers.MlpBlock_Real)' % (in_features, out_features))
        if not 1 <= depth_of_mlp <= _lib.FGNN_MAX_DEPTH:
            raise RuntimeError('depth_of_mlp must be in 1..%d' % _lib.FGNN_MAX_DEPTH)
        if original_features_num not in (2, 32):
            raise RuntimeError('the fused engine is built for original_features_num = 2 or 32 (got %d); other widths run '
                               'through the per-layer modules (layers.MlpBlock_Real)' % original_features_num)
        self.c0 = original_features_num
        self.num_blocks = num_blocks
        self.depth = depth_of_mlp
        self.entries = []
        self.mlp = {}
        off = 0
        last = original_features_num
        for blk in range(1, num_blocks + 1):
            for j, cin in ((1, last), (2, last), (3, last + 32)):
                pfx = 'ne_bm_block%d_mlp%d.' % (blk, j)
                rec = {'off': off, 'cin': cin, 'w': [], 'b': []}
                c = cin
                for i in range(depth_of_mlp):
                    self.entries.append((pfx + 'convs.%d.weight' % i, off, (32, c, 1, 1)))
                    rec['w'].append(off)
                    off += 32 * c
                    self.entries.append((pfx + 'convs.%d.bias' % i, off, (32,)))
                    rec['b'].append(off)
                    off += 32
                    c = 32
                self.entries.append((pfx + 'gn.weight', off, (1, 32, 1, 1)))
                rec['gn_w'] = off
                off += 32
                self.entries.append((pfx + 'gn.bias', off, (1, 32, 1, 1)))
                rec['gn_b'] = off
                off += 32
                rec['count'] = _lib.mlp_param_count(cin, depth_of_mlp)
                self.mlp[(blk, j)] = rec
            last = 32
        self.total = off

    def flatten(self, state_dict, device):
        flat = torch.empty(self.total, dtype=torch.float32, device=device)
        for name, off, shape in self.entries:
            key = name if name in state_dict else 'node_embedder.' + name
            t = state_dict[key]
            n = t.numel()
            flat[off:off + n].copy_(t.reshape(-1).to(torch.float32))
        return flat

    def init_flat(self, seed, device):
        gen = torch.Generator().manual_seed(seed)
        flat = torch.zeros(self.total, dtype=torch.float32)
        for name, off, shape in self.entries:
            n = _numel(shape)
            if name.endswith('.weight') and '.convs.' in name:
                fan_out, fan_in = shape[0], shape[1]
                bound = (6.0 / (fan_in + fan_out)) ** 0.5
                flat[off:off + n] = (torch.rand(n, generator=gen) * 2 - 1) * bound
            elif name.endswith('gn.weight'):
                flat[off:off + n] = 1.0
        return flat.to(device)

    def unflatten(self, flat):
        return {name: flat[off:off + _numel(shape)].view(shape) for name, off, shape in self.entries}


def _numel(shape):
    n = 1
    for s in shape:
        n *= s
    return n


def _round_up(x, m):
    return (x + m - 1) // m * m


class EngineCache:

    def __init__(self, budget):
        import collections
        self.budget = budget
        self._items = collections.OrderedDict()

    @staticmethod
    def engine_bytes(G, N, num_blocks, elt=4):
        ldp = -(-N * N // 32) * 32
        return (4 * num_blocks + 5) * G * 32 * ldp * elt

    def get(self, key, factory, nbytes):
        hit = self._items.get(key)
        if hit is not None:
            self._items.move_to_end(key)
            return hit[0], []
        eng = factory()
        self._items[key] = (eng, nbytes)
        evicted = []
        while self.used() > self.budget and len(self._items) > 1:
            k, _ = self._items.popitem(last=False)
            evicted.append(k)
        return eng, evicted

    def used(self):
        return sum(b for _, b in self._items.values())

    def keys(self):
        return list(self._items)

    def clear(self):
        self._items.clear()

    def __len__(self):
        return len(self._items)

    def __iter__(self):
        return iter(list(self._items))

    def values(self):
        return [e for e, _ in self._items.values()]


class FgnnEngine(EngineBase):
    SKIP_PADDING_TILES = True
    MM_ORDER = True
    PAIR_BWD = os.environ.get('FGNN_PAIR_BWD', '1') != '0'
    PACK_IN_STRUCT = os.environ.get('FGNN_PACK_IN_STRUCT', '1') != '0'
    T16 = os.environ.get('FGNN_T16', 'pair,bwd')

    MFMA = os.environ.get('FGNN_MFMA', 'f32')

    BLOCK1 = os.environ.get('FGNN_BLOCK1', 'generic')
    GN_FINALIZE = ('fgnn_gn_finalize', 'fgnn_gn_finalize2')

    def __init__(self, layout, G, N, device, ragged=False, cu_share=0, mfma=None, block1=None):
        _lib.load()
        self.T16 = type(self).T16
        self.cu_share = int(cu_share)
        mfma = self.MFMA if mfma is None else mfma
        if mfma not in ('f32', 'x3'):
            raise ValueError("mfma must be 'f32' or 'x3' (got %r)" % (mfma,))
        self.x3 = (mfma == 'x3' and not ragged and layout.depth == 3 and layout.c0 in (2, 32))
        block1 = self.BLOCK1 if block1 is None else block1
        if block1 not in ('generic', 'structured'):
            raise ValueError("block1 must be 'generic' or 'structured' (got %r)" % (block1,))
        self.struct1 = (block1 == 'structured' and cu_share == 0
                        and bool(_lib.load().fgnn_block1_struct_supported(N, layout.depth, layout.c0)))
        super().__init__(layout, G, N, device, ragged)
        self.P = N * N
        self.ldp = _round_up(self.P, 32)
        self.tpg = _lib.tiles_per_graph(N)
        self._gn_args = (EPS,)
        K = layout.num_blocks
        f32 = dict(dtype=torch.float32, device=device)
        self._act = act = lambda: torch.empty(G * 32 * self.ldp, **f32)
        self.z = {(k, j): act() for k in range(1, K + 1) for j in (1, 2, 3)}
        self.mult = {k: act() for k in range(1, K + 1)}
        self.part = [torch.empty(G * self.tpg * 32 * 2, **f32) for _ in range(2)]
        self.cnt = torch.empty(G * 2 * self.tpg, **f32)
        self.mm_order = (torch.empty(G, dtype=torch.int32, device=device)
                         if self.ranges is not None and self.MM_ORDER and 64 < N <= 256 else None)
        self.x = None
        self.xdeg = None
        self._packs = {}
        self._pack_entry = 'fgnn_pack_x3_operands' if self.x3 else 'fgnn_pack_operands'
        for k in range(1, K + 1):
            cin = layout.c0 if k == 1 else 32
            fl = _lib.load().fgnn_pack_x3_floats if self.x3 else _lib.load().fgnn_pack_floats
            f12, b12 = 0, (5 if self._t16_pair(cin) else 1)
            f3 = 2 if self.x3 else 0
            b3 = 5 if self._t16_bwd3(cin) else (3 if self.x3 else 1)
            self._packs[('f', k, 12)] = (f12, cin, 0, 2, torch.empty(fl(f12, cin, 0, layout.depth, 2), **f32))
            self._packs[('f', k, 3)] = (f3, 32, cin, 1, torch.empty(fl(f3, 32, cin, layout.depth, 1), **f32))
            for j in (1, 2):
                self._packs[('b', k, j)] = (b12, cin, 0, 1, torch.empty(fl(b12, cin, 0, layout.depth, 1), **f32))
            self._packs[('b', k, 3)] = (b3, 32, cin, 1, torch.empty(fl(b3, 32, cin, layout.depth, 1), **f32))

    def _t16(self, what):
        return self.T16 not in ('0', '') and what in self.T16.split(',')

    def _t16_pair(self, cin):
        return (self._t16('pair') and self.PAIR_BWD and not self.x3 and self.layout.depth == 3 and cin == 32 and self.N <= 256)

    def _t16_bwd3(self, cin):
        return self._t16('bwd') and not self.x3 and self.layout.depth == 3 and cin in (2, 32) and self.N <= 256

    def _slab_in(self, k, params):
        if k == 1:
            if self.xbits is not None:
                s = _lib.Slab()
                s.gstride, s.ldp, s.C = self.layout.c0 * self.P, self.P, self.layout.c0
                return s
            return _lib.make_slab(self.x, self.layout.c0 * self.P, self.P, self.layout.c0)
        rec = self.layout.mlp[(k - 1, 3)]
        s = _lib.make_slab(self.z[(k - 1, 3)], 32 * self.ldp, self.ldp, 32, nrm=self.nrm[(k - 1, 3)])
        s.beta = self._w(params, rec['gn_b'])
        return s

    def _slab_z(self, k, j, params):
        rec = self.layout.mlp[(k, j)]
        s = _lib.make_slab(self.z[(k, j)], 32 * self.ldp, self.ldp, 32, nrm=self.nrm[(k, j)])
        s.beta = self._w(params, rec['gn_b'])
        return s

    def _slab_raw(self, t):
        return _lib.make_slab(t, 32 * self.ldp, self.ldp, 32)

    def _mlp_fwd(self, params, k, js, a, b, finalize=True):
        L = self.layout
        args = _lib.MlpFwdArgs()
        args.G, args.N, args.depth, args.nmlp = self.G, self.N, L.depth, len(js)
        args.nvalid = self.nvalid.data_ptr() if self.nvalid is not None else None
        args.a = a
        if b is not None:
            args.b = b
        for m, j in enumerate(js):
            rec = L.mlp[(k, j)]
            for l in range(L.depth):
                args.W[m][l] = self._w(params, rec['w'][l])
                args.bias[m][l] = self._w(params, rec['b'][l])
            args.z[m] = self.z[(k, j)].data_ptr()
            args.part[m] = self.part[m].data_ptr()
        args.ldz = self.ldp
        args.cnt = self.cnt.data_ptr()
        args.packed = self._packs[('f', k, 12 if len(js) == 2 else 3)][4].data_ptr()
        self._packed_input(args, k)
        if self.ranges is not None:
            args.ranges = self.ranges.data_ptr()
        args.cu_share = self.cu_share
        st = _lib.stream_ptr()
        entry = 'fgnn_mlp_fwd_x3' if (self.x3 and len(js) == 2) else 'fgnn_mlp_fwd'
        _lib.call(entry, C.byref(args), st, tag='mlp_fwd[cin=%d,nmlp=%d]' % (a.C + (b.C if b is not None else 0), len(js)))
        if self.decisions is not None:
            bufs = [torch.zeros(self.G * (L.depth - 1) * 32 * self.tpg, dtype=torch.int32, device=self.device) for _ in js]
            _lib.call('fgnn_debug_mlp_fwd_x3_masks' if (self.x3 and len(js) == 2) else 'fgnn_debug_mlp_fwd_masks', C.byref(args),
                      _lib.ptr(bufs[0]), _lib.ptr(bufs[1]) if len(js) == 2 else None, st)
            for j, buf in zip(js, bufs):
                self.decisions[(k, j)] = buf
        if finalize:
            self._gn_finalize(params, k, js)

    def _packed_input(self, args, k):
        if k == 1 and self.xbits is not None:
            args.xbits = self.xbits.data_ptr()
            args.xdeg = self.xdeg.data_ptr()

    def embed(self, params, x, nvalid=None, bits=None, pack=True):
        L = self.layout
        self._adopt_nvalid(nvalid)
        st = _lib.stream_ptr()
        if self.ranges is not None:
            _lib.call('fgnn_ragged_tile_ranges_order', _lib.ptr(self.nvalid), self.G, self.N, _lib.ptr(self.ranges),
                      _lib.ptr(self.mm_order) if self.mm_order is not None else None, st, tag='fgnn_ragged_tile_ranges')
        if bits is not None:
            if x is not None or L.c0 != 2 or L.depth != 3:
                raise RuntimeError('FgnnEngine.embed: bits= replaces x and needs original_features_num = 2, depth_of_mlp = 3')
            self._check_bits(bits)
            if self.xdeg is None:
                self.xdeg = torch.empty(self.G * self.N, dtype=torch.float32, device=self.device)
            self.x, self.xbits = None, bits
            if not self.struct1:
                _lib.call('fgnn_adjacency_degree', _lib.ptr(bits), self._nv(), self.G, self.N, _lib.ptr(self.xdeg), st)
        else:
            if x.shape != (self.G, L.c0, self.N, self.N) or not x.is_contiguous() or x.dtype != torch.float32:
                raise RuntimeError('FgnnEngine.embed: expected contiguous fp32 %s, got %s %s'
                                   % ((self.G, L.c0, self.N, self.N), tuple(x.shape), x.dtype))
            self.x, self.xbits = x, None
        struct_now = self.struct1 and self.xbits is not None
        pack_in_struct = pack and struct_now and self.PACK_IN_STRUCT and not self.x3 and len(self._packs) <= _lib.MAX_PACK_JOBS
        if pack and not pack_in_struct:
            self.pack_operands(params)
        for k in range(1, L.num_blocks + 1):
            sin = self._slab_in(k, params)
            if k == 1 and struct_now:
                self._struct_fwd(params, with_pack=pack_in_struct)
                pool_fin = L.num_blocks == 1 and bool(_lib.load().fgnn_colmax_fwd_fin_supported(self.N))
                self._mlp_fwd(params, 1, (3,), self._slab_raw(self.mult[1]), sin, finalize=not pool_fin)
                continue
            fin = bool(_lib.load().fgnn_chan_matmul_fwd_fin_supported(self.N)) and self.G * 32 <= 4096
            self._mlp_fwd(params, k, (1, 2), sin, None, finalize=not fin)
            ya, yb = self._slab_z(k, 1, params), self._slab_z(k, 2, params)
            if fin:
                r1, r2 = L.mlp[(k, 1)], L.mlp[(k, 2)]
                _lib.call('fgnn_chan_matmul_fwd_fin_ord', C.byref(ya), C.byref(yb), _lib.ptr(self.part[0]), _lib.ptr(self.part[1]),
                          _lib.ptr(self.cnt), C.c_void_p(self._w(params, r1['gn_w'])), C.c_void_p(self._w(params, r2['gn_w'])),
                          EPS, self._nv(), self.G, self.N, _lib.ptr(self.mult[k]), 32 * self.ldp, self.ldp,
                          _lib.ptr(self.mm_order) if self.mm_order is not None else None, self._fill(), st, tag='fgnn_chan_matmul_fwd')
            else:
                _lib.call('fgnn_chan_matmul_fwd_ord', C.byref(ya), C.byref(yb), self._nv(), self.G, self.N,
                          _lib.ptr(self.mult[k]), 32 * self.ldp, self.ldp,
                          _lib.ptr(self.mm_order) if self.mm_order is not None else None, self._fill(), st, tag='fgnn_chan_matmul_fwd')
            pool_fin = k == L.num_blocks and bool(_lib.load().fgnn_colmax_fwd_fin_supported(self.N))
            self._mlp_fwd(params, k, (3,), self._slab_raw(self.mult[k]), sin, finalize=not pool_fin)
        out = self._slab_z(L.num_blocks, 3, params)
        if pool_fin:
            rec = L.mlp[(L.num_blocks, 3)]
            _lib.call('fgnn_colmax_fwd_fin', C.byref(out), _lib.ptr(self.part[0]), _lib.ptr(self.cnt),
                      C.c_void_p(self._w(params, rec['gn_w'])), EPS, self._nv(), self.G, self.N, _lib.ptr(self.E),
                      _lib.ptr(self.idx), st, tag='fgnn_colmax_fwd')
        else:
            _lib.call('fgnn_colmax_fwd', C.byref(out), self._nv(), self.G, self.N, _lib.ptr(self.E), _lib.ptr(self.idx), st)
        return self.E

    def _fill(self):
        return 1 if self.ranges is not None else 0

    def _struct_fwd(self, params, with_pack=False):
        S = self._struct_ws()
        st = _lib.stream_ptr()
        (w1, b1), (w2, b2) = self._w3(params, 1), self._w3(params, 2)
        r1, r2 = self.layout.mlp[(1, 1)], self.layout.mlp[(1, 2)]
        args = [_lib.ptr(self.xbits), self._nv(), self.G, self.N, _lib.ptr(S['tab']),
                C.c_void_p(self._w(params, r1['gn_w'])), C.c_void_p(self._w(params, r1['gn_b'])),
                C.c_void_p(self._w(params, r2['gn_w'])), C.c_void_p(self._w(params, r2['gn_b'])), EPS,
                _lib.ptr(self.nrm[(1, 1)]), _lib.ptr(self.nrm[(1, 2)]), _lib.ptr(self.mult[1]), 32 * self.ldp, self.ldp,
                _lib.ptr(self.xdeg), _lib.ptr(S['ws']), w1, b1, w2, b2]
        if with_pack:
            items = list(self._packs.items())
            _lib.call('fgnn_block1_struct_fwd_pack', *args, self._pack_jobs(params, items), len(items), st)
        else:
            _lib.call('fgnn_block1_struct_fwd', *args, st)

    def _struct_bwd(self, params):
        S, W = self._struct_ws(), self._bwd
        W['struct_rows'] = int(_lib.load().fgnn_block1_struct_rows(self.G, self.N))
        (w1, _), (w2, _) = self._w3(params, 1), self._w3(params, 2)
        r1, r2 = self.layout.mlp[(1, 1)], self.layout.mlp[(1, 2)]
        _lib.call('fgnn_block1_struct_bwd', _lib.ptr(self.xbits), self._nv(), self.G, self.N, _lib.ptr(S['tab']), w1, w2,
                  _lib.ptr(self.nrm[(1, 1)]), _lib.ptr(self.nrm[(1, 2)]),
                  C.c_void_p(self._w(params, r1['gn_b'])), C.c_void_p(self._w(params, r2['gn_b'])),
                  _lib.ptr(W['dmult']), 32 * self.ldp, self.ldp, _lib.ptr(S['ws']),
                  _lib.ptr(W['wpart'][(1, 1)]), _lib.ptr(W['wpart'][(1, 2)]), _lib.ptr(W['s12'][(1, 1)]), _lib.ptr(W['s12'][(1, 2)]),
                  _lib.stream_ptr())

    def _partial_rows(self):
        nwg = super()._partial_rows()
        if self.cu_share == 2 and self.ranges is None:
            nwg //= 2
        return nwg

    def _coef(self, kj, slot):
        W = self._bwd
        _lib.call('fgnn_gn_bwd_coef', _lib.ptr(W['s12'][kj]), _lib.ptr(self.nrm[kj]), self._nv(), self.G, 32, self.N,
                  _lib.ptr(W['coef'][slot]), None, None, _lib.stream_ptr())

    def _mlp_bwd(self, params, k, j, a, b, dy, coef, dxa, dxb, acc_a, acc_b, emit=False, dx_strides=None):
        args = self._mlp_bwd_args(params, k, j, a, b, dy, coef, dxa, dxb, acc_a, acc_b, emit, dx_strides)
        entry = 'fgnn_mlp_bwd_x3' if (self.x3 and j != 3) else 'fgnn_mlp_bwd'
        if j == 3 and b is not None and self._t16_bwd3(b.C) and _lib.load().fgnn_mlp_bwd_t16_supported(C.byref(args)):
            entry = 'fgnn_mlp_bwd_t16'
        elif self._packs[('b', k, j)][0] == 5:
            args.packed = None
        _lib.call(entry, C.byref(args), _lib.stream_ptr(),
                  tag='mlp_bwd[cin=%d,dx=%d]' % (a.C + (b.C if b is not None else 0),
                                                (a.C if dxa is not None else 0) + (b.C if (b is not None and dxb is not None) else 0)))

    def _mlp_bwd_pair(self, params, k, sin, din, emit):
        W = self._bwd
        a1 = self._mlp_bwd_args(params, k, 1, sin, None, W['dy1'], None, None, None, False, False, False, None)
        a2 = self._mlp_bwd_args(params, k, 2, sin, None, W['dy2'], None, din, None, True, False, emit, None)
        entry = 'fgnn_mlp_bwd_pair_x3' if self.x3 else ('fgnn_mlp_bwd_pair_t16' if self._t16_pair(sin.C) else 'fgnn_mlp_bwd_pair')
        _lib.call(entry, C.byref(a1), C.byref(a2), _lib.stream_ptr(),
                  tag='mlp_bwd_pair[cin=%d,dx=%d]' % (sin.C, sin.C if din is not None else 0))

    def _mlp_bwd_args(self, params, k, j, a, b, dy, coef, dxa, dxb, acc_a, acc_b, emit, dx_strides):
        L = self.layout
        W = self._bwd
        rec = L.mlp[(k, j)]
        gs = 32 * self.ldp
        args = _lib.MlpBwdArgs()
        args.G, args.N, args.depth = self.G, self.N, L.depth
        args.nvalid = self.nvalid.data_ptr() if self.nvalid is not None else None
        args.a = a
        if b is not None:
            args.b = b
        for l in range(L.depth):
            args.W[l] = self._w(params, rec['w'][l])
            args.bias[l] = self._w(params, rec['b'][l])
        args.dy, args.dgstride, args.ldd = dy.data_ptr(), gs, self.ldp
        args.z, args.zgstride, args.ldz = self.z[(k, j)].data_ptr(), gs, self.ldp
        if isinstance(coef, str):
            args.s12tiles = W['s12part'].data_ptr()
            args.s12_out = W['s12'][(k, j)].data_ptr()
            args.znrm = self.nrm[(k, j)].data_ptr()
        elif coef is not None:
            args.coef = coef.data_ptr()
        else:
            args.s12 = W['s12'][(k, j)].data_ptr()
            args.znrm = self.nrm[(k, j)].data_ptr()
        dgs, dld = (gs, self.ldp) if dx_strides is None else dx_strides
        if dxa is not None:
            args.dxa, args.dxa_gstride, args.dxa_ld = dxa.data_ptr(), (gs if (b is not None and dx_strides is not None) else dgs), \
                (self.ldp if (b is not None and dx_strides is not None) else dld)
        if dxb is not None:
            args.dxb, args.dxb_gstride, args.dxb_ld = dxb.data_ptr(), dgs, dld
        args.accumulate_a, args.accumulate_b = int(acc_a), int(acc_b)
        args.wpart = W['wpart'][(k, j)].data_ptr()
        args.packed = self._packs[('b', k, j)][4].data_ptr()
        self._packed_input(args, k)
        if self.ranges is not None:
            args.ranges = self.ranges.data_ptr()
        args.cu_share = self.cu_share
        if emit:
            args.s12part = W['s12part'].data_ptr()
        return args

    def backward_from_dE(self, params, grads, dE, finalize=True, dx=None):
        L = self.layout
        W = self._alloc_bwd()
        st = _lib.stream_ptr()
        gs = 32 * self.ldp
        K = L.num_blocks
        in_prologue = bool(_lib.load().fgnn_mlp_bwd_coef_tiles_supported(self.G, self.N)) and self.ranges is None
        dy = W['dy'][0]
        out = self._slab_z(K, 3, params)
        _lib.call('fgnn_colmax_bwd', _lib.ptr(dE), _lib.ptr(self.idx), self._nv(), self.G, 32, self.N,
                  _lib.ptr(dy), gs, self.ldp, C.byref(out), _lib.ptr(W['s12'][(K, 3)]), st)
        for k in range(K, 0, -1):
            sin = self._slab_in(k, params)
            first = (k == 1)
            din = None if first else W['dy'][(K - k + 1) % 2]
            dxs = None
            if first and dx is not None:
                if self.xbits is not None or self.x3 or tuple(dx.shape) != (self.G, L.c0, self.N, self.N) or dx.dtype != torch.float32 \
                        or not dx.is_contiguous():
                    raise RuntimeError('FgnnEngine: the input gradient needs a dense fp32 input, the fp32-MFMA kernels (mfma="f32") '
                                       'and a contiguous (G, c0, N, N) fp32 dx')
                din, dxs = dx, (L.c0 * self.P, self.P)
            self._mlp_bwd(params, k, 3, self._slab_raw(self.mult[k]), sin, dy,
                          None if k == K else ('tiles' if in_prologue else W['coef'][2]), W['dmult'], din, False, False, dx_strides=dxs)
            if first and self.struct1 and self.xbits is not None and dxs is None:
                self._struct_bwd(params)
                dy = din
                continue
            ya, yb = self._slab_z(k, 1, params), self._slab_z(k, 2, params)
            _lib.call('fgnn_chan_matmul_bwd_ord', C.byref(ya), C.byref(yb), _lib.ptr(W['dmult']), gs, self.ldp,
                      self._nv(), self.G, self.N, _lib.ptr(W['dy1']), _lib.ptr(W['dy2']), gs, self.ldp,
                      _lib.ptr(W['s12'][(k, 1)]), _lib.ptr(W['s12'][(k, 2)]),
                      _lib.ptr(self.mm_order) if self.mm_order is not None else None, self._fill(), st, tag='fgnn_chan_matmul_bwd')
            if first:
                W['struct_rows'] = 0
            if self.PAIR_BWD and dxs is None and L.depth == 3 and sin.C in (2, 32):
                self._mlp_bwd_pair(params, k, sin, din, emit=not first)
            else:
                self._mlp_bwd(params, k, 1, sin, None, W['dy1'], None, din, None, True, False, dx_strides=dxs)
                self._mlp_bwd(params, k, 2, sin, None, W['dy2'], None, din, None, True, False, emit=not first, dx_strides=dxs)
            if not first and not in_prologue:
                _lib.call('fgnn_gn_bwd_coef_tiles', _lib.ptr(W['s12part']), _lib.ptr(self.nrm[(k - 1, 3)]), self._nv(),
                          self.G, 32, self.N, _lib.ptr(W['s12'][(k - 1, 3)]), _lib.ptr(W['coef'][2]), st)
            dy = din
        if finalize:
            self.grad_finalize(grads)
        return grads

    def relu_decisions(self, params=None):
        L, G, N, P = self.layout, self.G, self.N, self.P
        out = {}
        bit = torch.arange(32, device=self.device, dtype=torch.int32)
        for (k, j), buf in self.decisions.items():
            w = buf.view(G, L.depth - 1, 32, self.tpg)
            m = ((w.unsqueeze(-1) >> bit) & 1).reshape(G, L.depth - 1, 32, self.tpg * 32)[..., :P].reshape(G, L.depth - 1, 32, N, N)
            for l in range(L.depth - 1):
                out[(k, j, l)] = m[:, l].bool()
        if self.struct1 and self.xbits is not None and (1, 1) not in self.decisions:
            nc = 2 + 2 * (N + 1)
            tab = self._struct['tab'].view(2, nc, 4, 32)
            words = (N + 31) // 32
            b = self.xbits.view(G, N, words).to(torch.int64) & 0xffffffff
            col = torch.arange(N, device=self.device)
            wmat = ((b[:, :, col // 32] >> (col % 32)) & 1)
            if self.nvalid is not None:
                nv = self.nvalid.to(torch.int64)
                inside = (col[None, :] < nv[:, None])
                wmat = wmat * (inside[:, :, None] & inside[:, None, :])
            deg = wmat.sum(-1)
            eye = torch.eye(N, device=self.device, dtype=torch.bool)
            diag_cls = 2 + 2 * deg + torch.diagonal(wmat, dim1=1, dim2=2)
            cls = torch.where(eye[None], diag_cls[:, :, None].expand(G, N, N), wmat)
            for j in (1, 2):
                for l in range(2):
                    hv = tab[j - 1, :, l, :] > 0
                    out[(1, j, l)] = hv[cls].permute(0, 3, 1, 2).contiguous()
        return out


    def normalized(self, k, j, params):
        rec = self.layout.mlp[(k, j)]
        y = torch.empty(self.G, 32, self.N, self.N, dtype=torch.float32, device=self.device)
        _lib.call('fgnn_gn_apply', _lib.ptr(self.z[(k, j)]), 32 * self.ldp, self.ldp, _lib.ptr(self.nrm[(k, j)]),
                  C.c_void_p(self._w(params, rec['gn_b'])), self._nv(), self.G, 32, self.N,
                  _lib.ptr(y), 32 * self.P, self.P, _lib.stream_ptr())
        return y

    def unpadded(self, buf):
        return buf.view(self.G, 32, self.ldp)[:, :, :self.P].reshape(self.G, 32, self.N, self.N).clone()
```

### include/fgnn_hip.h

```cpp
#ifndef FGNN_HIP_H
#define FGNN_HIP_H

#ifdef __cplusplus
extern "C" {
#endif

#define FGNN_H 32
#define FGNN_TILE 32
#define FGNN_MAX_DEPTH 3

typedef struct {
    const float *ptr;
    long long gstride;
    long long ldp;
    int C;
    const float *nrm;
    const float *beta;
} fgnn_slab;

const char *fgnn_last_error(void);
int fgnn_version(void);
int fgnn_tiles_per_graph(int N);
int fgnn_mlp_bwd_num_workgroups(void);

#define FGNN_MAX_PACK_JOBS 24
typedef struct {
    int kind, ca, cb, depth, nmlp;
    const float *W[2][FGNN_MAX_DEPTH];
    const float *bias[2][FGNN_MAX_DEPTH];
    float *out;
} fgnn_pack_job;
int fgnn_pack_floats(int kind, int ca, int cb, int depth, int nmlp);
int fgnn_pack_operands(const fgnn_pack_job *jobs, int njobs, void *stream);

typedef struct {
    int G, N, depth, nmlp;
    const int *nvalid;
    fgnn_slab a, b;
    const float *W[2][FGNN_MAX_DEPTH];
    const float *bias[2][FGNN_MAX_DEPTH];
    float *z[2];
    long long ldz;
    float *part[2];
    float *cnt;
    const float *packed;
    const unsigned *xbits;
    const float *xdeg;
    const int *ranges;
    int cu_share;
} fgnn_mlp_fwd_args;
int fgnn_mlp_fwd(const fgnn_mlp_fwd_args *args, void *stream);

int fgnn_pack_x3_floats(int kind, int ca, int cb, int depth, int nmlp);
int fgnn_pack_x3_operands(const fgnn_pack_job *jobs, int njobs, void *stream);
int fgnn_mlp_fwd_x3(const fgnn_mlp_fwd_args *args, void *stream);

int fgnn_gn_finalize(const float *part, const float *cnt, const float *gn_weight ,
                     const int *nvalid, int G, int C, int N, float eps, float *nrm, void *stream);
int fgnn_gn_finalize2(const float *part0, const float *part1, const float *cnt, const float *gn_weight0,
                      const float *gn_weight1, const int *nvalid, int G, int C, int N, float eps,
                      float *nrm0, float *nrm1, void *stream);
int fgnn_gn_stats(const float *x, long long gstride, long long ldp, const float *gn_weight,
                  const int *nvalid, int G, int C, int N, float eps, float *nrm, void *stream);
int fgnn_gn_apply(const float *z, long long zgstride, long long ldz, const float *nrm, const float *beta ,
                  const int *nvalid, int G, int C, int N, float *y, long long ygstride, long long ldy, void *stream);

int fgnn_gn_plane_supported(int N);
int fgnn_gn_plane_fwd(const float *x, long long gstride, long long ldp, const float *gn_weight, const float *beta ,
                      const int *nvalid, int G, int C, int N, float eps, float *y, long long ygstride, long long ldy,
                      float *nrm , void *stream);
int fgnn_gn_plane_bwd(const float *dy, long long dgstride, long long ldd, const float *z, long long zgstride, long long ldz,
                      const float *nrm, const int *nvalid, int G, int C, int N, float *dz, long long ogstride, long long ldo,
                      float *s12 , float *dgn_w , float *dgn_b , void *stream);

#define FGNN_CONV_MAX_CH 256
int fgnn_conv1x1(const float *x, long long x_gstride, long long x_ld, const float *relu_mask, const float *W,
                 long long w_ostride, long long w_kstride, const float *bias, int relu, const int *nvalid, int G, int N,
                 int M, int K, float *y, long long y_gstride, long long y_ld, void *stream);
int fgnn_conv1x1_dw_chunks(int G, int N);
int fgnn_conv1x1_dw(const float *dy, long long d_gstride, long long d_ld, const float *relu_mask, const float *x,
                    long long x_gstride, long long x_ld, const int *nvalid, int G, int N, int M, int K, float *wpart,
                    void *stream);

#define FGNN_DW_MAX_JOBS 4
typedef struct {
    const float *dy; long long d_gstride, d_ld;
    const float *relu_mask;
    const float *x; long long x_gstride, x_ld;
    int M, K;
} fgnn_dw_job;
int fgnn_conv1x1_dw_multi(const fgnn_dw_job *jobs, int njobs, const int *nvalid, int G, int N, float *wpart, void *stream);

typedef struct {
    const float *W;
    long long w_ostride, w_kstride;
    const float *bias;
    int M, K;
    int relu;
    const float *mask;
    float *out;
    long long o_gstride;
} fgnn_chain_layer;
typedef struct {
    const float *x;
    long long x_gstride, x_ld;
    int depth;
    fgnn_chain_layer layer[3];
    long long o_ld;
    const int *nvalid;
    int G, N;
} fgnn_chain_args;
int fgnn_conv_chain_supported(int depth, int K0, const int *M );
int fgnn_conv_chain(const fgnn_chain_args *args, void *stream);

typedef struct {
    const float *x;
    long long x_gstride, x_ld;
    int cin;
    const float *xb;
    long long xb_gstride, xb_ld;
    int cb;
    const float *packed;
    const int *nvalid;
    int G, N;
    float *out;
    long long o_gstride, o_ld;
    const float *dz;
    long long dz_gstride, dz_ld;
    float *dx;
    long long dx_gstride, dx_ld;
    float *dxb;
    long long dxb_gstride, dxb_ld;
    int accumulate_dx, accumulate_dxb;
    float *wpart;
} fgnn_mlp64_args;
int fgnn_mlp64_supported(int cin, int depth, int width);
int fgnn_mlp64_num_workgroups(void);
int fgnn_mlp64_param_count(int cin);
int fgnn_mlp64_packed_floats(int cin);
int fgnn_mlp64_pack(const float *W0, const float *W1, const float *W2, const float *b0, const float *b1, const float *b2, int cin,
                    float *packed, void *stream);
typedef struct {
    const float *W[3];
    const float *bias[3];
    int cin;
    float *packed;
} fgnn_mlp64_pack_job;
int fgnn_mlp64_pack_multi(const fgnn_mlp64_pack_job *jobs, int njobs, void *stream);
int fgnn_mlp64_fwd(const fgnn_mlp64_args *args, void *stream);
int fgnn_mlp64_bwd(const fgnn_mlp64_args *args, void *stream);

int fgnn_chan_matmul_fwd(const fgnn_slab *ya, const fgnn_slab *yb, const int *nvalid, int G, int N,
                         float *out, long long ogstride, long long ldo, void *stream);
int fgnn_chan_matmul_fwd_ord(const fgnn_slab *ya, const fgnn_slab *yb, const int *nvalid, int G, int N,
                             float *out, long long ogstride, long long ldo, const int *order, int fill, void *stream);
int fgnn_chan_matmul_fwd_fin_supported(int N);
int fgnn_chan_matmul_fwd_fin(const fgnn_slab *ya, const fgnn_slab *yb, const float *part_a, const float *part_b,
                             const float *cnt, const float *gn_weight_a, const float *gn_weight_b, float eps,
                             const int *nvalid, int G, int N, float *out, long long ogstride, long long ldo, void *stream);
int fgnn_chan_matmul_fwd_fin_ord(const fgnn_slab *ya, const fgnn_slab *yb, const float *part_a, const float *part_b,
                                 const float *cnt, const float *gn_weight_a, const float *gn_weight_b, float eps,
                                 const int *nvalid, int G, int N, float *out, long long ogstride, long long ldo,
                                 const int *order , int fill, void *stream);

int fgnn_colmax_fwd(const fgnn_slab *y, const int *nvalid, int G, int N, float *e ,
                    int *idx , void *stream);
int fgnn_colmax_fwd_fin_supported(int N);
int fgnn_colmax_fwd_fin(const fgnn_slab *y, const float *part, const float *cnt, const float *gn_weight, float eps,
                        const int *nvalid, int G, int N, float *e, int *idx, void *stream);

#define FGNN_SCORE_SPLIT 4
int fgnn_score_ce_fwd(const float *e1, const float *e2, const int *nvalid, int B, int C, int N,
                      float *scores, float *lse, float *pair_loss, void *stream);
int fgnn_score_row_blocks(int B, int N);
int fgnn_score_ce_fwd_blocks(const float *e1, const float *e2, const int *nvalid, int B, int C, int N, int row_blocks,
                             float *scores, float *lse, float *pair_loss, void *stream);
int fgnn_score_ce_bwd(const float *e1, const float *e2, const float *scores, const float *lse,
                      const int *nvalid, const float *gscale, int B, int C, int N,
                      float *de1, float *de2, void *stream);

int fgnn_ce_fwd(const float *scores, const int *nvalid, int B, int N, float *lse, float *pair_loss, void *stream);
int fgnn_ce_bwd(const float *scores, const float *lse, const int *nvalid, const float *gscale, int B, int N,
                float *dscores, void *stream);
int fgnn_score_bwd(const float *e1, const float *e2, const float *dscores, const int *nvalid,
                   int B, int C, int N, float *de1, float *de2, void *stream);

int fgnn_colmax_bwd(const float *de, const int *idx, const int *nvalid, int G, int C, int N,
                    float *dy, long long gstride, long long ldp, const fgnn_slab *y, float *s12, void *stream);

int fgnn_gn_bwd_stats(const float *dy, long long dgstride, long long ldd,
                      const float *z, long long zgstride, long long ldz, const float *nrm,
                      const int *nvalid, int G, int C, int N, float *s12 , void *stream);
int fgnn_gn_bwd_coef(const float *s12, const float *nrm, const int *nvalid, int G, int C, int N,
                     float *coef , float *dgn_w , float *dgn_b ,
                     void *stream);
int fgnn_gn_bwd_coef_tiles(const float *s12part, const float *nrm, const int *nvalid, int G, int C, int N,
                           float *s12, float *coef, void *stream);
int fgnn_gn_bwd_apply(const float *dy, long long dgstride, long long ldd,
                      const float *z, long long zgstride, long long ldz, const float *coef,
                      const int *nvalid, int G, int C, int N, float *dz, long long ogstride, long long ldo, void *stream);

typedef struct {
    int G, N, depth;
    const int *nvalid;
    fgnn_slab a, b;
    const float *W[FGNN_MAX_DEPTH];
    const float *bias[FGNN_MAX_DEPTH];
    const float *dy;  long long dgstride, ldd;
    const float *z;   long long zgstride, ldz;
    const float *coef;
    const float *s12;
    const float *znrm;
    float *dxa; long long dxa_gstride, dxa_ld;
    float *dxb; long long dxb_gstride, dxb_ld;
    int accumulate_a, accumulate_b;
    float *wpart;
    float *s12part;
    const float *packed;
    const float *s12tiles;
    float *s12_out;
    const unsigned *xbits;
    const float *xdeg;
    const int *ranges;
    int cu_share;
} fgnn_mlp_bwd_args;
int fgnn_mlp_bwd(const fgnn_mlp_bwd_args *args, void *stream);
int fgnn_mlp_bwd_x3(const fgnn_mlp_bwd_args *args, void *stream);
int fgnn_mlp_bwd_pair(const fgnn_mlp_bwd_args *m1, const fgnn_mlp_bwd_args *m2, void *stream);
int fgnn_mlp_bwd_pair_x3(const fgnn_mlp_bwd_args *m1, const fgnn_mlp_bwd_args *m2, void *stream);
int fgnn_mlp_bwd_t16_supported(const fgnn_mlp_bwd_args *args);
int fgnn_mlp_bwd_t16(const fgnn_mlp_bwd_args *args, void *stream);
int fgnn_mlp_bwd_pair_t16(const fgnn_mlp_bwd_args *m1, const fgnn_mlp_bwd_args *m2, void *stream);
#define FGNN_BWD_COEF_GRAPHS 4
int fgnn_mlp_bwd_coef_tiles_supported(int G, int N);
int fgnn_mlp_param_count(int Cin, int depth);
int fgnn_reduce_partials(const float *wpart, int num_wg, int count, float *out, void *stream);

#define FGNN_MAX_GRAD_JOBS 16
typedef struct {
    const float *wpart; int count; float *out;
    const float *s12; const float *nrm; float *dgn_w; float *dgn_b;
    int rows;
    float scale;
    const float *scale_dev;
} fgnn_grad_job;
int fgnn_grad_finalize(const fgnn_grad_job *jobs, int njobs, int num_wg, int G, int C, void *stream);
int fgnn_inv_node_count(const int *nvalid, int B, float *out, void *stream);

int fgnn_chan_matmul_bwd(const fgnn_slab *ya, const fgnn_slab *yb, const float *dm, long long dmgstride, long long ldm,
                         const int *nvalid, int G, int N,
                         float *da, float *db, long long ogstride, long long ldo,
                         float *s12a ,
                         float *s12b , void *stream);
int fgnn_chan_matmul_bwd_ord(const fgnn_slab *ya, const fgnn_slab *yb, const float *dm, long long dmgstride, long long ldm,
                             const int *nvalid, int G, int N, float *da, float *db, long long ogstride, long long ldo,
                             float *s12a, float *s12b, const int *order, int fill , void *stream);

int fgnn_adam_step(float *params, const float *grads, float *exp_avg, float *exp_avg_sq, int n, double lr,
                   double beta1, double beta2, double eps, int step, double grad_scale, void *stream);
int fgnn_adam_step_dev(float *params, const float *grads, float *exp_avg, float *exp_avg_sq, int n,
                       const double *hp, int *state, void *stream);
int fgnn_accuracy_max(const float *scores, const int *nvalid, int B, int N, int *correct, void *stream);
#define FGNN_LSAP_MAX_N 2048
int fgnn_lsap_accuracy(const float *cost, long long bstride, int ld, const int *nvalid, int B, int N, int *correct,
                       int *assign , void *stream);

int fgnn_block1_struct_supported(int N, int depth, int original_features_num);
int fgnn_block1_struct_table_floats(int N);
long long fgnn_block1_struct_ws_floats(int G, int N);
int fgnn_block1_struct_rows(int G, int N);
int fgnn_block1_struct_fwd(const unsigned *bits, const int *nvalid, int G, int N, const float *tables, const float *gnw1, const float *gnb1,
                           const float *gnw2, const float *gnb2, float eps, float *nrm1, float *nrm2, float *mult, long long gstride,
                           long long ldp, float *xdeg , float *ws,
                           const float *const *tW1, const float *const *tb1, const float *const *tW2, const float *const *tb2
                           ,
                           void *stream);
int fgnn_block1_struct_bwd(const unsigned *bits, const int *nvalid, int G, int N, const float *tables, const float *const *W1,
                           const float *const *W2, const float *nrm1, const float *nrm2, const float *gnb1, const float *gnb2,
                           const float *dmult, long long gstride, long long ldp, float *ws, float *wpart1, float *wpart2, float *s12_1,
                           float *s12_2, void *stream);
int fgnn_block1_struct_fwd_pack(const unsigned *bits, const int *nvalid, int G, int N, const float *tables, const float *gnw1, const float *gnb1,
                                const float *gnw2, const float *gnb2, float eps, float *nrm1, float *nrm2, float *mult, long long gstride,
                                long long ldp, float *xdeg, float *ws, const float *const *tW1, const float *const *tb1,
                                const float *const *tW2, const float *const *tb2, const fgnn_pack_job *jobs, int njobs, void *stream);
int fgnn_block1_struct_fwd16(const unsigned *bits, const int *nvalid, int G, int N, int ldr, const float *tables, const float *gnw1,
                             const float *gnb1, const float *gnw2, const float *gnb2, float eps, float *nrm1, float *nrm2,
                             void *mult , long long gstride, long long ldp, void *x16 , float *ws,
                             const float *const *tW1, const float *const *tb1, const float *const *tW2, const float *const *tb2, void *stream);
int fgnn_block1_struct_fwd16_pack(const unsigned *bits, const int *nvalid, int G, int N, int ldr, const float *tables, const float *gnw1,
                                  const float *gnb1, const float *gnw2, const float *gnb2, float eps, float *nrm1, float *nrm2, void *mult,
                                  long long gstride, long long ldp, void *x16, float *ws, const float *const *tW1, const float *const *tb1,
                                  const float *const *tW2, const float *const *tb2, const fgnn_pack_job *jobs, int njobs, void *stream);
int fgnn_block1_struct_bwd16(const unsigned *bits, const int *nvalid, int G, int N, int ldr, const float *tables, const float *const *W1,
                             const float *const *W2, const float *nrm1, const float *nrm2, const float *gnb1, const float *gnb2,
                             const void *dmult , long long gstride, long long ldp, float *ws, float *wpart1, float *wpart2,
                             float *s12_1, float *s12_2, void *stream);

int fgnn_expand_adjacency(const unsigned *bits, const int *nvalid, int G, int N, float *x, void *stream);
int fgnn_pack_adjacency(const float *x, const int *nvalid, int G, int N, unsigned *bits, int *bad, void *stream);
int fgnn_pack_adjacency_ld(const float *x, const int *nvalid, int G, int Nin, int N, unsigned *bits, int *bad, void *stream);
int fgnn_pack_adjacency_pair(const float *x1, const float *x2, const int *nvalid1, const int *nvalid2, int B, int Nin, int N, unsigned *bits,
                             int *nv_out, float *inv_out, int *bad, void *stream);
int fgnn_adjacency_degree(const unsigned *bits, const int *nvalid, int G, int N, float *deg, void *stream);

#define FGNN_RANGE_WG 256
int fgnn_ragged_tile_ranges(const int *nvalid, int G, int N, int *ranges , void *stream);
int fgnn_ragged_tile_ranges_order(const int *nvalid, int G, int N, int *ranges , int *order ,
                                  void *stream);
int fgnn_ragged_tile_ranges16(const int *nvalid, int G, int N, int ldr, int *ranges , void *stream);

int fgnn_sum_scale(const float *in, int rows, int cols, float scale, float *out, void *stream);

typedef struct {
    const void *ptr;
    long long gstride;
    long long ldp;
    int C;
    const float *nrm;
    const float *beta;
} fgnn_slab16;
int fgnn_tiles_per_graph16(int N, int ldr);

int fgnn_to_bf16(const float *x, const int *nvalid, int G, int C, int N, int ldr, void *y, long long gstride, long long ldp,
                 void *stream);
int fgnn_from_bf16(const void *y, long long gstride, long long ldp, int G, int C, int N, int ldr, float *x, void *stream);

int fgnn_pack16_floats(int kind, int ca, int cb, int depth, int nmlp);
int fgnn_pack16_operands(const fgnn_pack_job *jobs, int njobs, void *stream);

typedef struct {
    int G, N, ldr, depth, nmlp;
    const int *nvalid;
    fgnn_slab16 a, b;
    void *z[2];
    long long ldz;
    float *part[2];
    float *cnt;
    const void *packed;
    const int *ranges;
} fgnn_mlp_fwd16_args;
int fgnn_mlp_fwd16(const fgnn_mlp_fwd16_args *args, void *stream);
int fgnn_debug_mlp_fwd16_masks(const fgnn_mlp_fwd16_args *args, unsigned *masks0, unsigned *masks1, void *stream);

int fgnn_gn_finalize_tpg(const float *part, const float *cnt, const float *gn_weight, const int *nvalid, int G, int C, int N,
                         int tpg, float eps, float *nrm, void *stream);
int fgnn_gn_finalize2_tpg(const float *part0, const float *part1, const float *cnt, const float *gn_weight0,
                          const float *gn_weight1, const int *nvalid, int G, int C, int N, int tpg, float eps, float *nrm0,
                          float *nrm1, void *stream);
int fgnn_gn_bwd_coef_tiles_tpg(const float *s12part, const float *nrm, const int *nvalid, int G, int C, int N, int tpg,
                               float *s12, float *coef, void *stream);

int fgnn_chan_matmul_fwd16(const fgnn_slab16 *ya, const fgnn_slab16 *yb, const int *nvalid, int G, int N, int ldr,
                           void *out, long long ogstride, long long ldo, void *stream);
int fgnn_chan_matmul_fwd16_fin(const fgnn_slab16 *ya, const fgnn_slab16 *yb, const float *part_a, const float *part_b,
                               const float *cnt, const float *gn_weight_a, const float *gn_weight_b, float eps, int tpg,
                               const int *nvalid, int G, int N, int ldr, void *out, long long ogstride, long long ldo,
                               void *stream);
int fgnn_chan_matmul_bwd16(const fgnn_slab16 *ya, const fgnn_slab16 *yb, const void *dm, long long dmgstride, long long ldm,
                           const int *nvalid, int G, int N, int ldr, void *da, void *db, long long ogstride, long long ldo,
                           float *s12a, float *s12b, void *stream);

int fgnn_chan_matmul_bwd16_t(const fgnn_slab16 *ya, const fgnn_slab16 *yb, const void *dm, long long dmgstride, long long ldm,
                             const float *tpart, int tpg, const int *nvalid, int G, int N, int ldr, void *da, void *db,
                             long long ogstride, long long ldo, float *s12a, float *s12b, void *stream);

int fgnn_chan_matmul_bwd16_tc(const fgnn_slab16 *ya, const fgnn_slab16 *yb, const void *dm, long long dmgstride, long long ldm,
                              const float *tpart, int tpg, const int *nvalid, int G, int N, int ldr, void *da, void *db,
                              long long ogstride, long long ldo, float *s12a, float *s12b, float *coefa, float *coefb,
                              void *stream);
int fgnn_colmax_fwd16(const fgnn_slab16 *y, const int *nvalid, int G, int N, int ldr, float *e, int *idx, void *stream);
int fgnn_colmax_bwd16(const float *de, const int *idx, const int *nvalid, int G, int C, int N, int ldr, void *dy,
                      long long gstride, long long ldp, const fgnn_slab16 *y, float *s12, void *stream);
int fgnn_colmax_bwd16_coef(const float *de, const int *idx, const int *nvalid, int G, int C, int N, int ldr, void *dy,
                           long long gstride, long long ldp, const fgnn_slab16 *y, float *s12, float *coef, void *stream);

typedef struct {
    int G, N, ldr, depth;
    const int *nvalid;
    fgnn_slab16 a, b;
    const void *dy;  long long dgstride, ldd;
    const void *z;   long long zgstride, ldz;
    const float *coef;
    void *dxa; long long dxa_gstride, dxa_ld;
    void *dxb; long long dxb_gstride, dxb_ld;
    int accumulate_a, accumulate_b;
    float *wpart;
    float *s12part;
    const void *packed;
    const int *ranges;
} fgnn_mlp_bwd16_args;
int fgnn_mlp_bwd16(const fgnn_mlp_bwd16_args *args, void *stream);
int fgnn_mlp_bwd16_pair(const fgnn_mlp_bwd16_args *m1, const fgnn_mlp_bwd16_args *m2, void *stream);

#define FGNN_PAIRGEN_ERDOS_RENYI 0
#define FGNN_PAIRGEN_REGULAR 1
#define FGNN_PAIRGEN_BARABASI_ALBERT 2
#define FGNN_PAIRGEN_EDGE_SWAP 1
#define FGNN_PAIRGEN_MAX_N 256
typedef struct {
    unsigned long long seed;
    long long first;
    int B, N;
    int family, noise_model;
    double edge_density;
    unsigned long long thr_edge;
    unsigned long long thr_noise1;
    unsigned long long thr_noise2;
    unsigned long long thr_vertex;
    int swaps_per_edge;
    unsigned *bits1, *bits2;
    int *nvalid;
} fgnn_pairgen_args;
int fgnn_pairgen_supported(int N, int family, int noise_model);
int fgnn_pairgen(const fgnn_pairgen_args *args, void *stream);

#define FGNN_QAP_MAX_N 256
int fgnn_qap_objective(const unsigned *bits1, const unsigned *bits2, const int *assign, const int *nvalid, int B, int N, int *qap,
                       int *planted, int *na, int *nb, void *stream);
int fgnn_qap_improve_cost(const unsigned *bits1, const unsigned *bits2, const int *assign, const int *nvalid, int B, int N, float *cost,
                          long long bstride, int ld, void *stream);
long long fgnn_greedy_qap_ws_bytes(int B, int N);
int fgnn_greedy_qap(const unsigned *bits1, const unsigned *bits2, const int *assign0, const int *nvalid, int B, int N, int T, void *ws,
                    long long ws_bytes, int *s_best2, int *acc_best, int *t_best, int *perm_best , void *stream);

#define FGNN_SPECTRAL_MAX_N 256
#define FGNN_SPECTRAL_MAX_POWERS 8
int fgnn_spectral_features(const unsigned *bits, const int *nvalid, int G, int N, int n_powers, float *out, int Nout, void *stream);

int fgnn_debug_mlp_fwd_masks(const fgnn_mlp_fwd_args *args, unsigned *masks0, unsigned *masks1 , void *stream);
int fgnn_debug_mlp_fwd_x3_masks(const fgnn_mlp_fwd_args *args, unsigned *masks0, unsigned *masks1, void *stream);
int fgnn_debug_matmul_variant(int wave_per_matrix);

#ifdef __cplusplus
}
#endif
#endif
```

Baseline: 42510.

## Replace dense colmax backward gradient with compact pooling records read by MLP backward

```diff
diff --git a/graph_neural_net_amd/_lib.py b/graph_neural_net_amd/_lib.py
--- a/graph_neural_net_amd/_lib.py
+++ b/graph_neural_net_amd/_lib.py
@@ -83,7 +83,7 @@
                 ('accumulate_a', C.c_int), ('accumulate_b', C.c_int),
                 ('wpart', C.c_void_p), ('s12part', C.c_void_p), ('packed', C.c_void_p),
                 ('s12tiles', C.c_void_p), ('s12_out', C.c_void_p), ('xbits', C.c_void_p), ('xdeg', C.c_void_p),
-                ('ranges', C.c_void_p), ('cu_share', C.c_int)]
+                ('ranges', C.c_void_p), ('cu_share', C.c_int), ('pool_rec', C.c_void_p)]
 
 
 class Slab16(C.Structure):
@@ -190,6 +190,9 @@
     'fgnn_ce_fwd': [_VP, _VP, _I, _I, _VP, _VP, _VP],
     'fgnn_ce_bwd': [_VP, _VP, _VP, _VP, _I, _I, _VP, _VP],
     'fgnn_colmax_bwd': [_VP, _VP, _VP, _I, _I, _I, _VP, _LL, _LL, C.POINTER(Slab), _VP, _VP],
+    'fgnn_pool_records': [_VP, _VP, _VP, _I, _I, C.POINTER(Slab), _VP, _VP, _VP],
+    'fgnn_score_ce_bwd_pool_supported': [_I, _I, _I],
+    'fgnn_score_ce_bwd_pool': [_VP, _VP, _VP, _VP, _VP, _VP, _I, _I, _I, _VP, _VP, _VP, C.POINTER(Slab), _VP, _VP, _VP],
     'fgnn_gn_bwd_stats': [_VP, _LL, _LL, _VP, _LL, _LL, _VP, _VP, _I, _I, _I, _VP, _VP],
     'fgnn_gn_bwd_coef': [_VP, _VP, _VP, _I, _I, _I, _VP, _VP, _VP, _VP],
     'fgnn_gn_bwd_coef_tiles': [_VP, _VP, _VP, _I, _I, _I, _VP, _VP, _VP],
diff --git a/graph_neural_net_amd/csrc/mlp_bwd_t16.hip b/graph_neural_net_amd/csrc/mlp_bwd_t16.hip
--- a/graph_neural_net_amd/csrc/mlp_bwd_t16.hip
+++ b/graph_neural_net_amd/csrc/mlp_bwd_t16.hip
@@ -7,6 +7,7 @@
 
 constexpr int BWD_WG = 256;
 constexpr int NW = 8;
+typedef unsigned u32x4 __attribute__((ext_vector_type(4)));
 
 DEVI float4 coef_from_sums(const float4 n, const float2 sv, float nv) {
     const float m = nv * nv;
@@ -42,7 +43,7 @@
     static constexpr int LDS_F = MAIN_F > RED_F ? MAIN_F : RED_F;
 };
 
-template <int CB, bool PKD, bool SKIP, bool DXB>
+template <int CB, bool PKD, bool SKIP, bool DXB, bool VDY = false>
 __global__ __launch_bounds__(64 * NW, 2) void mlp_bwd_t16_kernel(const fgnn_mlp_bwd_args A, const int tpg, const int total_tiles) {
     extern __shared__ __attribute__((aligned(16))) float smem[];
     using L = Layout16<CB>;
@@ -55,6 +56,7 @@
     PackedSrc ps = {};
     if constexpr (PKD) ps = make_packed_src(A.xbits, A.xdeg, A.G, A.N);
     const View vdy = make_view(A.dy, A.dgstride, A.ldd, A.G);
+    const rsrc_t rrec = __builtin_amdgcn_make_buffer_rsrc(const_cast<void *>(A.pool_rec), 0, VDY ? A.G * A.N * 256 : 0, 0x00020000);
     const View vz = make_view(A.z, A.zgstride, A.ldz, A.G);
     const View vdxa = make_view(A.dxa, A.dxa_gstride, A.dxa_ld, A.G);
     const View vdxb = make_view(A.dxb, A.dxb_gstride, A.dxb_ld, A.G);
@@ -176,6 +178,7 @@
 
     constexpr int NXB = CB == 32 ? 8 : 1;
     float xa[8], xb[NXB], dyr[8], zr[8];
+    u32x4 prr[4];
     auto load_x = [&](int h) {
         const bool act = h < H1;
         const int g = __builtin_amdgcn_readfirstlane(act ? h / hpg : 0);
@@ -201,7 +204,15 @@
         const int g = __builtin_amdgcn_readfirstlane(act ? h / hpg : 0);
         const int p = (act ? h - g * hpg : 0) * 16 + px;
         const bool inb = act && p < P2;
-        load8(dyr, vdy, lane_voff(vdy, q, p, inb), g * vdy.gs4);
+        if constexpr (VDY) {
+            int i, jj;
+            row_col(p, A.N, rcpN, i, jj);
+            const int voff = inb ? i * 256 + q * 64 : OOB_OFF;
+#pragma unroll
+            for (int k = 0; k < 4; ++k) prr[k] = __builtin_amdgcn_raw_buffer_load_b128(rrec, voff, g * A.N * 256 + 16 * k, 0);
+        } else {
+            load8(dyr, vdy, lane_voff(vdy, q, p, inb), g * vdy.gs4);
+        }
         load8(zr, vz, lane_voff(vz, q, p, inb), g * vz.gs4);
     };
 
@@ -311,6 +322,15 @@
             stage8(S1, lane_base, h2);
         }
         float dpre[8];
+        if constexpr (VDY) {
+            int i, jj;
+            row_col(p, A.N, rcpN, i, jj);
+#pragma unroll
+            for (int s = 0; s < 8; ++s) {
+                const unsigned de = prr[s >> 1][2 * (s & 1)], bi = prr[s >> 1][2 * (s & 1) + 1];
+                dyr[s] = jj == (int)bi ? __builtin_bit_cast(float, de) : 0.f;
+            }
+        }
 #pragma unroll
         for (int s = 0; s < 8; ++s) dpre[s] = fmaf(kz[s], zr[s] - kx[s], fmaf(ky[s], dyr[s], kw[s]));
         if (!full) {
@@ -433,20 +453,20 @@
     }
 }
 
-template <int CB, bool PKD, bool SKIP, bool DXB>
+template <int CB, bool PKD, bool SKIP, bool DXB, bool VDY = false>
 int launch16(const fgnn_mlp_bwd_args *a, int tpg, int total, hipStream_t st) {
     constexpr int LDS = Layout16<CB>::LDS_F * 4;
     static_assert(LDS <= 160 * 1024, "LDS budget");
     static LdsAttrCache attr_cache;
-    (void)fgnn_raise_lds(attr_cache, (const void *)mlp_bwd_t16_kernel<CB, PKD, SKIP, DXB>, LDS);
-    hipLaunchKernelGGL((mlp_bwd_t16_kernel<CB, PKD, SKIP, DXB>), dim3(a->cu_share == 2 && !SKIP ? BWD_WG / 2 : BWD_WG), dim3(64 * NW), LDS, st, *a,
+    (void)fgnn_raise_lds(attr_cache, (const void *)mlp_bwd_t16_kernel<CB, PKD, SKIP, DXB, VDY>, LDS);
+    hipLaunchKernelGGL((mlp_bwd_t16_kernel<CB, PKD, SKIP, DXB, VDY>), dim3(a->cu_share == 2 && !SKIP ? BWD_WG / 2 : BWD_WG), dim3(64 * NW), LDS, st, *a,
                        tpg, total);
     FGNN_LAUNCH_CHECK();
     return 0;
 }
-template <int CB, bool PKD, bool DXB>
+template <int CB, bool PKD, bool DXB, bool VDY = false>
 int launch16s(const fgnn_mlp_bwd_args *a, int tpg, int total, hipStream_t st) {
-    return a->ranges ? launch16<CB, PKD, true, DXB>(a, tpg, total, st) : launch16<CB, PKD, false, DXB>(a, tpg, total, st);
+    return a->ranges ? launch16<CB, PKD, true, DXB, VDY>(a, tpg, total, st) : launch16<CB, PKD, false, DXB, VDY>(a, tpg, total, st);
 }
 
 }
@@ -454,6 +474,7 @@
 extern "C" int fgnn_mlp_bwd_t16_supported(const fgnn_mlp_bwd_args *a) {
     if (!a || a->depth != 3 || a->a.C != 32 || a->a.nrm || !a->dxa || a->accumulate_a || a->accumulate_b || !a->packed || a->N > 256) return 0;
     if (a->b.C == 32) return (a->b.nrm && a->dxb && !a->xbits) ? 1 : 0;
+    if (a->pool_rec) return 0;
     if (a->b.C == 2) return (!a->b.nrm && !a->dxb) ? 1 : 0;
     return 0;
 }
@@ -461,15 +482,16 @@
 extern "C" int fgnn_mlp_bwd_t16(const fgnn_mlp_bwd_args *a, void *stream) {
     FGNN_CHECK(a != nullptr, "fgnn_mlp_bwd_t16: null args");
     FGNN_CHECK(fgnn_mlp_bwd_t16_supported(a), "fgnn_mlp_bwd_t16: built for depth 3, slab a = 32 raw channels with dx stored, slab b = 32 normalised "
-               "channels with dx stored or 2 raw channels without dx, an operand image of kind 5, N <= 256; use fgnn_mlp_bwd");
+               "channels with dx stored or 2 raw channels without dx (and no pool_rec), an operand image of kind 5, N <= 256; use fgnn_mlp_bwd");
     FGNN_CHECK(a->G > 0 && a->N > 0 && a->a.ptr && (a->b.ptr || (a->xbits && a->b.C == 2)), "fgnn_mlp_bwd_t16: bad G / N / slabs");
     FGNN_CHECK(!a->xbits || a->xdeg, "fgnn_mlp_bwd_t16: xbits without xdeg (fgnn_adjacency_degree)");
-    FGNN_CHECK(a->dy && a->z && a->wpart, "fgnn_mlp_bwd_t16: missing dy/z/wpart");
+    FGNN_CHECK((a->dy || a->pool_rec) && a->z && a->wpart, "fgnn_mlp_bwd_t16: missing dy/z/wpart");
+    FGNN_CHECK(!a->pool_rec || (long long)a->G * a->N * 256 < 0x7fffffffll, "fgnn_mlp_bwd_t16: pool_rec exceeds 2 GiB; split the batch");
     FGNN_CHECK(a->coef || (a->s12 && a->znrm) || (a->s12tiles && a->znrm), "fgnn_mlp_bwd_t16: need coef, or s12 + znrm, or s12tiles + znrm");
     FGNN_CHECK(BWD_WG == fgnn_mlp_bwd_num_workgroups() && BWD_WG == FGNN_RANGE_WG, "fgnn_mlp_bwd_t16: workgroup count differs from fgnn_mlp_bwd");
     {
         const long long lim = 0x7fffffffll / 4, G = a->G;
-        FGNN_CHECK(G * a->a.gstride < lim && G * a->b.gstride < lim && G * a->dgstride < lim && G * a->zgstride < lim &&
+        FGNN_CHECK(G * a->a.gstride < lim && G * a->b.gstride < lim && (a->pool_rec || G * a->dgstride < lim) && G * a->zgstride < lim &&
                    G * a->dxa_gstride < lim && G * a->dxb_gstride < lim,
                    "fgnn_mlp_bwd_t16: a tensor exceeds 2 GiB (32-bit buffer addressing); split the batch");
     }
@@ -481,6 +503,7 @@
     FGNN_CHECK(!a->s12tiles || fgnn_mlp_bwd_coef_tiles_supported(a->G, a->N), "fgnn_mlp_bwd_t16: s12tiles needs a workgroup's tile range to span <= %d graphs",
                FGNN_BWD_COEF_GRAPHS);
     hipStream_t st = (hipStream_t)stream;
+    if (a->b.C == 32 && a->pool_rec) return launch16s<32, false, true, true>(a, tpg, (int)total, st);
     if (a->b.C == 32) return launch16s<32, false, true>(a, tpg, (int)total, st);
     if (a->xbits) return launch16s<2, true, false>(a, tpg, (int)total, st);
     return launch16s<2, false, false>(a, tpg, (int)total, st);
diff --git a/graph_neural_net_amd/csrc/pool_score.hip b/graph_neural_net_amd/csrc/pool_score.hip
--- a/graph_neural_net_amd/csrc/pool_score.hip
+++ b/graph_neural_net_amd/csrc/pool_score.hip
@@ -281,6 +281,44 @@
     }
 }
 
+struct __attribute__((aligned(8))) PoolRec {
+    float de;
+    int idx;
+};
+__global__ __launch_bounds__(256) void pool_records_kernel(const float *de, const int *idx, const int *nvalid, int C, int N,
+                                                           const fgnn_slab y, PoolRec *rec, float *s12) {
+    __shared__ float red[4][2];
+    const int gc = blockIdx.x, tid = threadIdx.x, lane = tid & 63, wave = tid >> 6;
+    const int g = gc / C, c = gc - g * C;
+    const int nv = nvalid_of(nvalid, g, N);
+    const float *zm = y.ptr + (long long)g * y.gstride + (long long)c * y.ldp;
+    const float mean = y.nrm[(long long)gc * 4];
+    float s1 = 0.f, s2 = 0.f;
+    if (tid < N) {
+        const long long t = (long long)gc * N + tid;
+        const int bi = idx[t];
+        const float d = tid < nv ? de[t] : 0.f;
+        float zv = 0.f;
+        if (tid < nv) zv = zm[(long long)tid * N + bi];
+        PoolRec r;
+        r.de = d;
+        r.idx = bi;
+        rec[((long long)g * N + tid) * 32 + FGNN_POOL_REC_POS(c)] = r;
+        if (tid < nv) {
+            s1 += d;
+            s2 += d * (zv - mean);
+        }
+    }
+    s1 = wave_sum(s1);
+    s2 = wave_sum(s2);
+    if (lane == 0) {
+        red[wave][0] = s1;
+        red[wave][1] = s2;
+    }
+    __syncthreads();
+    if (tid < 2) s12[(long long)gc * 2 + tid] = (red[0][tid] + red[1][tid]) + (red[2][tid] + red[3][tid]);
+}
+
 DEVI void copy_to_lds256(float *dst, const float *src, int n, int tid) {
     constexpr int U = 8;
     int done = 0;
@@ -371,10 +409,16 @@
 
 constexpr int CSPLIT = 4;
 constexpr int CSPLIT_SMALL = 8;
-template <bool CE, bool STAGE>
+struct PoolOut {
+    const int *idx;
+    fgnn_slab y;
+    PoolRec *rec;
+    float *s12;
+};
+template <bool CE, bool STAGE, bool POOL = false>
 __global__ __launch_bounds__(256) void score_bwd_kernel(const float *e1, const float *e2, const float *scores,
                                                         const float *lse, const float *dscores, const int *nvalid,
-                                                        const float *gscale, int C, int N, float *de1, float *de2) {
+                                                        const float *gscale, int C, int N, float *de1, float *de2, const PoolOut PO) {
     extern __shared__ __attribute__((aligned(16))) float sm[];
     const int cper = (C + (int)gridDim.y - 1) / (int)gridDim.y;
     const int c0 = blockIdx.y * cper;
@@ -423,9 +467,31 @@
             }
         }
     }
+    const int B = gridDim.x;
+    int bi_first[2] = {0, 0};
+    if constexpr (POOL) {
+        if (tid < cn * N) {
+            bi_first[0] = PO.idx[((long long)b * C + c0) * N + tid];
+            bi_first[1] = PO.idx[((long long)(B + b) * C + c0) * N + tid];
+        }
+    }
     __syncthreads();
+    float *pst = dS + (STAGE ? N * ld : 0);
     for (int e = tid; e < cn * N; e += 256) {
         const int c = e / N, i = e - c * N;
+        int bi[2] = {0, 0};
+        float zv[2] = {0.f, 0.f}, mean[2] = {0.f, 0.f};
+        int nvg[2] = {nv, nv};
+        if constexpr (POOL) {
+#pragma unroll
+            for (int h = 0; h < 2; ++h) {
+                const int g = h * B + b;
+                nvg[h] = nvalid_of(nvalid, g, N);
+                bi[h] = e == tid ? bi_first[h] : PO.idx[((long long)g * C + c0) * N + e];
+                mean[h] = PO.y.nrm[((long long)g * C + c0 + c) * 4];
+                if (i < nvg[h]) zv[h] = PO.y.ptr[(long long)g * PO.y.gstride + (long long)(c0 + c) * PO.y.ldp + (long long)i * N + bi[h]];
+            }
+        }
         float a1 = 0.f, a2 = 0.f;
         if (i < nv) {
             const float *r2 = s2 + c * N, *r1 = s1 + c * N;
@@ -436,6 +502,46 @@
         }
         de1[((long long)b * C + c0) * N + e] = a1;
         de2[((long long)b * C + c0) * N + e] = a2;
+        if constexpr (POOL) {
+#pragma unroll
+            for (int h = 0; h < 2; ++h) {
+                const int g = h * B + b;
+                const float d = i < nvg[h] ? (h ? a2 : a1) : 0.f;
+                PoolRec r;
+                r.de = d;
+                r.idx = bi[h];
+                PO.rec[((long long)g * N + i) * 32 + FGNN_POOL_REC_POS(c0 + c)] = r;
+                pst[((h * cper + c) * N + i) * 2] = d;
+                pst[((h * cper + c) * N + i) * 2 + 1] = d * (zv[h] - mean[h]);
+            }
+        }
+    }
+    if constexpr (POOL) {
+        const int lane = tid & 63, wave = __builtin_amdgcn_readfirstlane(tid >> 6);
+        float *red = pst + 4 * cper * N;
+        __syncthreads();
+        for (int t = wave; t < 2 * cn * 4; t += 4) {
+            const int w = t & 3, hc = t >> 2, h = hc / cn, c = hc - h * cn;
+            const int i = w * 64 + lane;
+            const int nvh = nvalid_of(nvalid, h * B + b, N);
+            float p1 = 0.f, p2 = 0.f;
+            if (i < N && i < nvh) {
+                p1 += pst[((h * cper + c) * N + i) * 2];
+                p2 += pst[((h * cper + c) * N + i) * 2 + 1];
+            }
+            p1 = wave_sum(p1);
+            p2 = wave_sum(p2);
+            if (lane == 0) {
+                red[((h * cper + c) * 4 + w) * 2] = p1;
+                red[((h * cper + c) * 4 + w) * 2 + 1] = p2;
+            }
+        }
+        __syncthreads();
+        if (tid < 2 * cn * 2) {
+            const int k = tid & 1, hc = tid >> 1, h = hc / cn, c = hc - h * cn;
+            const float *r = red + (h * cper + c) * 8 + k;
+            PO.s12[((long long)(h * B + b) * C + c0 + c) * 2 + k] = (r[0] + r[2]) + (r[4] + r[6]);
+        }
     }
 }
 
@@ -622,19 +728,27 @@
     const int cper = (C + csplit - 1) / csplit;
     return (2 * cper * N + (stage ? N * (N + 1) : 0)) * (int)sizeof(float);
 }
+static bool score_bwd_stages(int B, int C, int N) {
+    return score_bwd_lds_bytes(C, N, true) <= 160 * 1024 && (N <= 64 || (long long)B * CSPLIT >= 256);
+}
+static int score_bwd_csplit(int B) { return (long long)B * CSPLIT < 256 ? CSPLIT_SMALL : CSPLIT; }
+static int score_bwd_pool_lds_bytes(int C, int N, int csplit) {
+    const int cper = (C + csplit - 1) / csplit;
+    return (4 * cper * N + 16 * cper) * (int)sizeof(float);
+}
 template <bool CE>
 static int launch_score_bwd(const float *e1, const float *e2, const float *scores, const float *lse,
                             const float *dscores, const int *nvalid, const float *gscale, int B, int C, int N,
                             float *de1, float *de2, hipStream_t st) {
-    const bool stage = score_bwd_lds_bytes(C, N, true) <= 160 * 1024 && (N <= 64 || (long long)B * CSPLIT >= 256);
-    const int csplit = (long long)B * CSPLIT < 256 ? CSPLIT_SMALL : CSPLIT;
+    const bool stage = score_bwd_stages(B, C, N);
+    const int csplit = score_bwd_csplit(B);
     const int lds = score_bwd_lds_bytes(C, N, stage, stage ? csplit : CSPLIT);
     FGNN_CHECK(lds <= 160 * 1024, "score backward: C*N=%d too large for LDS staging", C * N);
     if (stage) {
         if (lds > 64 * 1024)
             (void)hipFuncSetAttribute((const void *)score_bwd_kernel<CE, true>, hipFuncAttributeMaxDynamicSharedMemorySize, lds);
         hipLaunchKernelGGL((score_bwd_kernel<CE, true>), dim3(B, csplit), dim3(256), lds, st, e1, e2, scores, lse, dscores,
-                           nvalid, gscale, C, N, de1, de2);
+                           nvalid, gscale, C, N, de1, de2, PoolOut{});
     } else {
         const int cper = (C + CSPLIT - 1) / CSPLIT;
         const int SB_BLK = (long long)B * CSPLIT * ((N + 63) / 64) >= 512 ? 64 : 16;
@@ -681,6 +795,41 @@
     return launch_score_bwd<true>(e1, e2, scores, lse, nullptr, nvalid, gscale, B, C, N, de1, de2, (hipStream_t)stream);
 }
 
+extern "C" int fgnn_score_ce_bwd_pool_supported(int B, int C, int N) {
+    if (B <= 0 || C != 32 || N <= 0 || N > 256 || !score_bwd_stages(B, C, N)) return 0;
+    const int csplit = score_bwd_csplit(B);
+    return score_bwd_lds_bytes(C, N, true, csplit) + score_bwd_pool_lds_bytes(C, N, csplit) <= 160 * 1024 ? 1 : 0;
+}
+
+extern "C" int fgnn_score_ce_bwd_pool(const float *e1, const float *e2, const float *scores, const float *lse, const int *nvalid,
+                                      const float *gscale, int B, int C, int N, float *de1, float *de2, const int *idx,
+                                      const fgnn_slab *y, void *rec, float *s12, void *stream) {
+    FGNN_CHECK(e1 && e2 && scores && lse && gscale && de1 && de2 && B > 0, "fgnn_score_ce_bwd_pool: bad arguments");
+    FGNN_CHECK(idx && rec && s12 && y && y->ptr && y->nrm && y->C == C, "fgnn_score_ce_bwd_pool: needs idx, rec, s12 and the normalised input slab");
+    FGNN_CHECK(fgnn_score_ce_bwd_pool_supported(B, C, N), "fgnn_score_ce_bwd_pool: built for C = 32, N <= 256 and the whole-dS form; use "
+               "fgnn_score_ce_bwd + fgnn_pool_records");
+    const int csplit = score_bwd_csplit(B);
+    const int lds = score_bwd_lds_bytes(C, N, true, csplit) + score_bwd_pool_lds_bytes(C, N, csplit);
+    static LdsAttrCache attr_cache;
+    (void)fgnn_raise_lds(attr_cache, (const void *)score_bwd_kernel<true, true, true>, lds);
+    const PoolOut po = {idx, *y, static_cast<PoolRec *>(rec), s12};
+    hipLaunchKernelGGL((score_bwd_kernel<true, true, true>), dim3(B, csplit), dim3(256), lds, (hipStream_t)stream, e1, e2, scores, lse,
+                       nullptr, nvalid, gscale, C, N, de1, de2, po);
+    FGNN_LAUNCH_CHECK();
+    return 0;
+}
+
+extern "C" int fgnn_pool_records(const float *de, const int *idx, const int *nvalid, int G, int N, const fgnn_slab *y, void *rec,
+                                 float *s12, void *stream) {
+    FGNN_CHECK(de && idx && rec && s12 && G > 0 && N > 0, "fgnn_pool_records: bad arguments");
+    FGNN_CHECK(N <= 256, "fgnn_pool_records: N=%d > 256 (use fgnn_colmax_bwd)", N);
+    FGNN_CHECK(y && y->ptr && y->nrm && y->C == 32, "fgnn_pool_records: needs the normalised 32-channel input slab of the pooling");
+    hipLaunchKernelGGL(pool_records_kernel, dim3((unsigned)(G * 32)), dim3(256), 0, (hipStream_t)stream, de, idx, nvalid, 32, N, *y,
+                       static_cast<PoolRec *>(rec), s12);
+    FGNN_LAUNCH_CHECK();
+    return 0;
+}
+
 extern "C" int fgnn_score_bwd(const float *e1, const float *e2, const float *dscores, const int *nvalid, int B, int C,
                               int N, float *de1, float *de2, void *stream) {
     FGNN_CHECK(e1 && e2 && dscores && de1 && de2 && B > 0, "fgnn_score_bwd: bad arguments");
diff --git a/graph_neural_net_amd/engine.py b/graph_neural_net_amd/engine.py
--- a/graph_neural_net_amd/engine.py
+++ b/graph_neural_net_amd/engine.py
@@ -138,6 +138,7 @@
     PAIR_BWD = os.environ.get('FGNN_PAIR_BWD', '1') != '0'
     PACK_IN_STRUCT = os.environ.get('FGNN_PACK_IN_STRUCT', '1') != '0'
     T16 = os.environ.get('FGNN_T16', 'pair,bwd')
+    VIRTUAL_DY = os.environ.get('FGNN_VIRTUAL_DY', '1') != '0'
 
     MFMA = os.environ.get('FGNN_MFMA', 'f32')
 
@@ -147,6 +148,7 @@
     def __init__(self, layout, G, N, device, ragged=False, cu_share=0, mfma=None, block1=None):
         _lib.load()
         self.T16 = type(self).T16
+        self.virtual_dy = type(self).VIRTUAL_DY
         self.cu_share = int(cu_share)
         mfma = self.MFMA if mfma is None else mfma
         if mfma not in ('f32', 'x3'):
@@ -355,11 +357,15 @@
         _lib.call('fgnn_gn_bwd_coef', _lib.ptr(W['s12'][kj]), _lib.ptr(self.nrm[kj]), self._nv(), self.G, 32, self.N,
                   _lib.ptr(W['coef'][slot]), None, None, _lib.stream_ptr())
 
-    def _mlp_bwd(self, params, k, j, a, b, dy, coef, dxa, dxb, acc_a, acc_b, emit=False, dx_strides=None):
+    def _mlp_bwd(self, params, k, j, a, b, dy, coef, dxa, dxb, acc_a, acc_b, emit=False, dx_strides=None, pool_rec=None):
         args = self._mlp_bwd_args(params, k, j, a, b, dy, coef, dxa, dxb, acc_a, acc_b, emit, dx_strides)
+        if pool_rec is not None:
+            args.pool_rec = pool_rec.data_ptr()
         entry = 'fgnn_mlp_bwd_x3' if (self.x3 and j != 3) else 'fgnn_mlp_bwd'
         if j == 3 and b is not None and self._t16_bwd3(b.C) and _lib.load().fgnn_mlp_bwd_t16_supported(C.byref(args)):
             entry = 'fgnn_mlp_bwd_t16'
+        elif pool_rec is not None:
+            raise RuntimeError('FgnnEngine: no kernel takes the pooling records for this launch')
         elif self._packs[('b', k, j)][0] == 5:
             args.packed = None
         _lib.call(entry, C.byref(args), _lib.stream_ptr(),
@@ -416,7 +422,43 @@
             args.s12part = W['s12part'].data_ptr()
         return args
 
-    def backward_from_dE(self, params, grads, dE, finalize=True, dx=None):
+    def _virtual_dy(self, params, dx=None):
+        K = self.layout.num_blocks
+        if not self.virtual_dy or dx is not None:
+            return False
+        W = self._alloc_bwd()
+        if 'virtual_ok' not in W:
+            sin = self._slab_in(K, params) if (K > 1 or self.x is not None or self.xbits is not None) else None
+            ok = sin is not None and sin.C == 32 and self._t16_bwd3(32)
+            if ok:
+                if 'pool_rec' not in W:
+                    W['pool_rec'] = torch.empty(self.G * self.N * 32 * 2, dtype=torch.float32, device=self.device)
+                args = self._mlp_bwd_args(params, K, 3, self._slab_raw(self.mult[K]), sin, W['dy'][0], None, W['dmult'],
+                                          W['dy'][1], False, False, False, None)
+                args.pool_rec = W['pool_rec'].data_ptr()
+                ok = bool(_lib.load().fgnn_mlp_bwd_t16_supported(C.byref(args)))
+            W['virtual_ok'] = ok
+        return W['virtual_ok']
+
+    def backward(self, params, grads, grad_scale=1.0, gscale_dev=None, **kw):
+        B, N = self.B, self.N
+        if not (self._virtual_dy(params, kw.get('dx')) and _lib.load().fgnn_score_ce_bwd_pool_supported(B, 32, N)):
+            return super().backward(params, grads, grad_scale, gscale_dev, **kw)
+        W = self._alloc_bwd()
+        gs_t = W['gscale']
+        if gscale_dev is not None:
+            gs_t = gscale_dev
+        else:
+            self._set_gscale(grad_scale / self.total_nodes)
+        e1, e2 = self.E[:B], self.E[B:]
+        out = self._slab_z(self.layout.num_blocks, 3, params)
+        _lib.call('fgnn_score_ce_bwd_pool', _lib.ptr(e1), _lib.ptr(e2), _lib.ptr(self.scores), _lib.ptr(self.lse),
+                  self._nv(), _lib.ptr(gs_t), B, 32, N, _lib.ptr(W['dE'][:B]), _lib.ptr(W['dE'][B:]), _lib.ptr(self.idx),
+                  C.byref(out), _lib.ptr(W['pool_rec']), _lib.ptr(W['s12'][(self.layout.num_blocks, 3)]), _lib.stream_ptr(),
+                  tag='fgnn_score_ce_bwd')
+        return self.backward_from_dE(params, grads, W['dE'], _records=True, **kw)
+
+    def backward_from_dE(self, params, grads, dE, finalize=True, dx=None, _records=False):
         L = self.layout
         W = self._alloc_bwd()
         st = _lib.stream_ptr()
@@ -425,8 +467,13 @@
         in_prologue = bool(_lib.load().fgnn_mlp_bwd_coef_tiles_supported(self.G, self.N)) and self.ranges is None
         dy = W['dy'][0]
         out = self._slab_z(K, 3, params)
-        _lib.call('fgnn_colmax_bwd', _lib.ptr(dE), _lib.ptr(self.idx), self._nv(), self.G, 32, self.N,
-                  _lib.ptr(dy), gs, self.ldp, C.byref(out), _lib.ptr(W['s12'][(K, 3)]), st)
+        virtual = self._virtual_dy(params, dx)
+        if not virtual:
+            _lib.call('fgnn_colmax_bwd', _lib.ptr(dE), _lib.ptr(self.idx), self._nv(), self.G, 32, self.N,
+                      _lib.ptr(dy), gs, self.ldp, C.byref(out), _lib.ptr(W['s12'][(K, 3)]), st)
+        elif not _records:
+            _lib.call('fgnn_pool_records', _lib.ptr(dE), _lib.ptr(self.idx), self._nv(), self.G, self.N, C.byref(out),
+                      _lib.ptr(W['pool_rec']), _lib.ptr(W['s12'][(K, 3)]), st)
         for k in range(K, 0, -1):
             sin = self._slab_in(k, params)
             first = (k == 1)
@@ -439,7 +486,8 @@
                                        'and a contiguous (G, c0, N, N) fp32 dx')
                 din, dxs = dx, (L.c0 * self.P, self.P)
             self._mlp_bwd(params, k, 3, self._slab_raw(self.mult[k]), sin, dy,
-                          None if k == K else ('tiles' if in_prologue else W['coef'][2]), W['dmult'], din, False, False, dx_strides=dxs)
+                          None if k == K else ('tiles' if in_prologue else W['coef'][2]), W['dmult'], din, False, False, dx_strides=dxs,
+                          pool_rec=W['pool_rec'] if (virtual and k == K) else None)
             if first and self.struct1 and self.xbits is not None and dxs is None:
                 self._struct_bwd(params)
                 dy = din
diff --git a/include/fgnn_hip.h b/include/fgnn_hip.h
--- a/include/fgnn_hip.h
+++ b/include/fgnn_hip.h
@@ -187,6 +187,13 @@
 
 int fgnn_colmax_bwd(const float *de, const int *idx, const int *nvalid, int G, int C, int N,
                     float *dy, long long gstride, long long ldp, const fgnn_slab *y, float *s12, void *stream);
+#define FGNN_POOL_REC_POS(c) (8 * (2 * ((c) & 1) + (((c) >> 2) & 1)) + 2 * ((c) >> 3) + (((c) >> 1) & 1))
+int fgnn_pool_records(const float *de, const int *idx, const int *nvalid, int G, int N, const fgnn_slab *y, void *rec, float *s12,
+                      void *stream);
+int fgnn_score_ce_bwd_pool_supported(int B, int C, int N);
+int fgnn_score_ce_bwd_pool(const float *e1, const float *e2, const float *scores, const float *lse, const int *nvalid,
+                           const float *gscale, int B, int C, int N, float *de1, float *de2, const int *idx, const fgnn_slab *y,
+                           void *rec, float *s12, void *stream);
 
 int fgnn_gn_bwd_stats(const float *dy, long long dgstride, long long ldd,
                       const float *z, long long zgstride, long long ldz, const float *nrm,
@@ -223,6 +230,7 @@
     const float *xdeg;
     const int *ranges;
     int cu_share;
+    const void *pool_rec;
 } fgnn_mlp_bwd_args;
 int fgnn_mlp_bwd(const fgnn_mlp_bwd_args *args, void *stream);
 int fgnn_mlp_bwd_x3(const fgnn_mlp_bwd_args *args, void *stream);
```

New measurement: 42830 (median of 6 runs). Within noise of the previous version (+0.7%).
